# YaoTiancheng/DirectComputeRayTracing

Hardware: AMD Instinct MI355X
Metric: Mrays/s and ms/spp at 1920x1080, 8-bounce wavefront (higher is better)
Workload: dtype f32; 1 GPU; cornell_box_obj 1920x1080, 1733 spp (1 spp/step, film stripes across 1 GPU(s)), 8 bounces, wavefront, point light; spp=1733, max_bounce=8, streams_per_gpu=3, snapshot_spp=1733, parallelism=single GPU, 3 concurrent pipelines per GPU (cost-balanced bands), partition=balanced, interleave=False, bands_per_rank=3, rays=48252902736

## Files before the change

### directcomputeraytracing_amd/_abi.py

```python
from __future__ import annotations

import ctypes as C
import os
from pathlib import Path

PKG_DIR = Path(__file__).resolve().parent
LIB_PATH = PKG_DIR / "libdcrt.so"

DCRT_OK = 0
ABI_VERSION = 5
ERRORS = {-1: "DCRT_E_INVALID_ARG", -2: "DCRT_E_HIP", -3: "DCRT_E_NO_SCENE", -4: "DCRT_E_IO",
          -5: "DCRT_E_LIMIT", -6: "DCRT_E_NO_DEVICE"}
LIGHT_INDEX_INVALID = 0xFFFFFFFF
FEATURE_GGX_SAMPLE_VNDF = 0x01
FEATURE_NO_FRONT_TO_BACK = 0x02
FEATURE_LIGHT_VISIBLE = 0x04
FEATURE_WATERTIGHT = 0x08
FEATURE_ALLOW_ANYHIT = 0x10
FEATURE_DEFAULT = FEATURE_GGX_SAMPLE_VNDF | FEATURE_LIGHT_VISIBLE | FEATURE_WATERTIGHT
FILTER_BOX, FILTER_TRIANGLE, FILTER_GAUSSIAN, FILTER_MITCHELL, FILTER_LANCZOS = range(5)
MATERIAL_DIFFUSE, MATERIAL_PLASTIC, MATERIAL_CONDUCTOR, MATERIAL_DIELECTRIC, MATERIAL_THIN_DIELECTRIC = range(5)
MAX_LIGHT_COUNT = 5000
DIRTY_LIGHTS = 0x01
DIRTY_MATERIALS = 0x02
DIRTY_INSTANCE_FLAGS = 0x04
DIRTY_CAMERA = 0x08
DIRTY_SCENE = 0x10
(OUTPUT_PATH_TRACING, OUTPUT_SHADING_NORMAL, OUTPUT_SHADING_TANGENT, OUTPUT_ALBEDO, OUTPUT_NEGATIVE_NDOTV,
 OUTPUT_BACKFACE, OUTPUT_ITERATION_COUNT) = range(7)


class Vertex(C.Structure):
    _fields_ = [("position", C.c_float * 3), ("normal", C.c_float * 3), ("tangent", C.c_float * 3),
                ("texcoord", C.c_float * 2)]


class BVHNode(C.Structure):
    _fields_ = [("bbox_min", C.c_float * 3), ("bbox_max", C.c_float * 3), ("right_child_or_prim_index", C.c_uint32),
                ("misc", C.c_uint32)]


class Material(C.Structure):
    _fields_ = [("albedo", C.c_float * 3), ("albedo_texture_index", C.c_int32), ("ior", C.c_float * 3),
                ("roughness", C.c_float), ("tex_tiling", C.c_float * 2), ("opacity", C.c_float),
                ("flags", C.c_uint32), ("opacity_texture_index", C.c_int32)]


class Light(C.Structure):
    _fields_ = [("radiance", C.c_float * 3), ("position_or_triangle_range", C.c_float * 3), ("flags", C.c_uint32)]


class Float4x3(C.Structure):
    _fields_ = [("m", C.c_float * 12)]


class Texture(C.Structure):
    _fields_ = [("width", C.c_uint32), ("height", C.c_uint32), ("format", C.c_uint32),
                ("pixels", C.POINTER(C.c_uint8))]


class FlatScene(C.Structure):
    _fields_ = [
        ("vertices", C.POINTER(Vertex)), ("vertex_count", C.c_uint32),
        ("triangles", C.POINTER(C.c_uint32)), ("triangle_count", C.c_uint32),
        ("bvh_nodes", C.POINTER(BVHNode)), ("bvh_node_count", C.c_uint32),
        ("tlas_node_count", C.c_uint32),
        ("material_ids", C.POINTER(C.c_uint32)),
        ("instance_transforms", C.POINTER(Float4x3)), ("instance_count", C.c_uint32),
        ("instance_light_indices", C.POINTER(C.c_uint32)),
        ("instance_flags", C.POINTER(C.c_uint32)),
        ("instance_material_overrides", C.POINTER(C.c_uint32)),
        ("materials", C.POINTER(Material)), ("material_count", C.c_uint32),
        ("lights", C.POINTER(Light)), ("light_count", C.c_uint32),
        ("environment_light_index", C.c_uint32),
        ("textures", C.POINTER(Texture)), ("texture_count", C.c_uint32),
        ("env_cube_rgb", C.POINTER(C.c_float)), ("env_cube_size", C.c_uint32),
        ("bvh_traversal_stack_size", C.c_uint32),
    ]


class BxDFLuts(C.Structure):
    _fields_ = [("brdf", C.c_uint16 * (32 * 32)), ("brdf_avg", C.c_uint16 * 32),
                ("brdf_dielectric", C.c_uint16 * (32 * 16 * 32)), ("brdf_dielectric_avg", C.c_uint16 * (16 * 16 * 2)),
                ("bsdf", C.c_uint16 * (32 * 16 * 32)), ("bsdf_avg", C.c_uint16 * (16 * 16 * 2))]


class FrameParams(C.Structure):
    _fields_ = [("camera_transform", C.c_float * 16), ("resolution", C.c_uint32 * 2), ("film_size", C.c_float * 2),
                ("aperture_radius", C.c_float), ("focal_distance", C.c_float), ("film_distance", C.c_float),
                ("blade_count", C.c_uint32), ("blade_vertex_pos", C.c_float * 2), ("aperture_base_angle", C.c_float),
                ("frame_seed", C.c_uint32), ("max_bounce_count", C.c_uint32), ("light_count", C.c_uint32),
                ("environment_light_index", C.c_uint32), ("features", C.c_uint32)]


class FilterParams(C.Structure):
    _fields_ = [("filter", C.c_uint32), ("radius", C.c_float), ("gaussian_alpha", C.c_float),
                ("mitchell_b", C.c_float), ("mitchell_c", C.c_float), ("lanczos_tau", C.c_uint32)]


class Ray(C.Structure):
    _fields_ = [("origin", C.c_float * 3), ("t_max", C.c_float), ("direction", C.c_float * 3), ("t_min", C.c_float)]


class RayHit(C.Structure):
    _fields_ = [("t", C.c_float), ("u", C.c_float), ("v", C.c_float), ("triangle_id", C.c_uint32),
                ("instance_index", C.c_uint32)]


class PostFxParams(C.Structure):
    _fields_ = [("enabled", C.c_int32), ("auto_exposure", C.c_int32), ("ev100", C.c_float), ("luminance_white", C.c_float)]


class TracerConfig(C.Structure):
    _fields_ = [("path_pool_size", C.c_uint32), ("iterations_per_render", C.c_uint32), ("device", C.c_int32),
                ("stream", C.c_void_p), ("debug_rng", C.c_uint32)]


class OutputParams(C.Structure):
    _fields_ = [("output_type", C.c_uint32), ("iteration_threshold", C.c_uint32)]


class DenoiseParams(C.Structure):
    _fields_ = [("iterations", C.c_uint32), ("sigma_luminance", C.c_float), ("sigma_normal", C.c_float),
                ("sigma_albedo", C.c_float), ("demodulate", C.c_uint32)]


class NoiseStats(C.Structure):
    _fields_ = [("images", C.c_uint32), ("valid_pixels", C.c_uint32), ("converged_pixels", C.c_uint32),
                ("mean_error", C.c_float), ("max_error", C.c_float), ("max_tile_error", C.c_float)]


class ConvergeParams(C.Structure):
    _fields_ = [("threshold", C.c_float), ("target_fraction", C.c_float), ("min_images", C.c_uint32),
                ("max_images", C.c_uint32), ("check_interval", C.c_uint32)]


class AdaptiveReport(C.Structure):
    _fields_ = [("images", C.c_uint32), ("check_points", C.c_uint32), ("pixel_samples", C.c_uint64),
                ("active_blocks", C.c_uint32), ("total_blocks", C.c_uint32)]


class RayStats(C.Structure):
    _fields_ = [("extension_rays", C.c_uint64), ("shadow_rays", C.c_uint64), ("new_paths", C.c_uint64),
                ("iterations", C.c_uint64), ("images_completed", C.c_uint64)]


class FilmPartition(C.Structure):
    _fields_ = [("world_size", C.c_uint32), ("rank", C.c_uint32), ("stripe_height", C.c_uint32),
                ("halo_rows", C.c_uint32)]


class TraversalStats(C.Structure):
    _fields_ = [("ext_node_visits", C.c_uint64), ("ext_triangle_tests", C.c_uint64), ("ext_blas_entries", C.c_uint64),
                ("shadow_node_visits", C.c_uint64), ("shadow_triangle_tests", C.c_uint64),
                ("shadow_blas_entries", C.c_uint64), ("ext_launches", C.c_uint64), ("ext_kernel_ms", C.c_double),
                ("ext_max_node_visits", C.c_uint64), ("shadow_max_node_visits", C.c_uint64),
                ("material_launches", C.c_uint64), ("material_kernel_ms", C.c_double),
                ("control_launches", C.c_uint64), ("control_kernel_ms", C.c_double)]


class TracerInfo(C.Structure):
    _fields_ = [("path_pool_size", C.c_uint32), ("scene_in_lds", C.c_uint32), ("cached_nodes", C.c_uint32),
                ("cached_triangles", C.c_uint32), ("cast_block", C.c_uint32), ("traversal_stack", C.c_uint32),
                ("material_generic", C.c_uint32), ("pair_traversal", C.c_uint32), ("control_grid", C.c_uint32),
                ("material_grid", C.c_uint32), ("cast_grid", C.c_uint32), ("material_lds", C.c_uint32),
                ("cast_identity", C.c_uint32), ("stack_lds_rows", C.c_uint32), ("ring_rows", C.c_uint32),
                ("cast_waves_per_cu", C.c_uint32), ("shadow_cells", C.c_uint32), ("shadow_cell_max_leaves", C.c_uint32),
                ("shadow_cell_mean_leaves", C.c_float), ("shadow_inline", C.c_uint32), ("shading_tables", C.c_uint32),
                ("dielectric_row_bytes", C.c_uint32), ("dielectric_row_lds", C.c_uint32), ("frame_table_bytes", C.c_uint32)]


class ShadowCellsInfo(C.Structure):
    _fields_ = [("resolution", C.c_uint32), ("leaf_count", C.c_uint32), ("node_count", C.c_uint32),
                ("max_leaves", C.c_uint32), ("mean_leaves", C.c_float), ("r0", C.c_float)]


class UploadStats(C.Structure):
    _fields_ = [("scene_uploads", C.c_uint64), ("material_updates", C.c_uint64), ("light_updates", C.c_uint64),
                ("instance_flag_updates", C.c_uint64), ("geometry_bytes", C.c_uint64), ("shading_bytes", C.c_uint64),
                ("graph_invalidations", C.c_uint64)]


class MaterialSetting(C.Structure):
    _fields_ = [("albedo", C.c_float * 3), ("roughness", C.c_float), ("ior", C.c_float * 3), ("opacity", C.c_float),
                ("k", C.c_float * 3), ("tiling", C.c_float * 2), ("material_type", C.c_uint32),
                ("albedo_texture_index", C.c_int32), ("opacity_texture_index", C.c_int32),
                ("internal_scattering_mode", C.c_uint32), ("multiscattering", C.c_uint32),
                ("is_two_sided", C.c_uint32), ("has_roughness_texture", C.c_uint32)]


class SceneSettings(C.Structure):
    _fields_ = [("resolution", C.c_uint32 * 2), ("max_bounce_count", C.c_uint32), ("camera_type", C.c_uint32),
                ("fov_x", C.c_float), ("focal_length", C.c_float), ("focal_distance", C.c_float),
                ("relative_aperture", C.c_float), ("aperture_blade_count", C.c_uint32), ("aperture_rotation", C.c_float),
                ("film_size", C.c_float * 2), ("camera_position", C.c_float * 3), ("camera_euler_angles", C.c_float * 3),
                ("features", C.c_uint32), ("has_environment_light", C.c_uint32), ("environment_color", C.c_float * 3),
                ("env_cube_rgb", C.POINTER(C.c_float)), ("env_cube_size", C.c_uint32),
                ("mesh_light_count", C.c_uint32), ("punctual_light_count", C.c_uint32),
                ("material_count", C.c_uint32), ("texture_count", C.c_uint32)]


class ObjMesh(C.Structure):
    _fields_ = [("vertices", C.POINTER(Vertex)), ("vertex_count", C.c_uint32), ("indices", C.POINTER(C.c_uint32)),
                ("material_ids", C.POINTER(C.c_uint32)), ("triangle_count", C.c_uint32)]


class ObjMaterial(C.Structure):
    _fields_ = [("albedo", C.c_float * 3), ("ior", C.c_float), ("roughness", C.c_float), ("opacity", C.c_float),
                ("albedo_texture_index", C.c_int32), ("opacity_texture_index", C.c_int32)]


class BsdfProbeMaterial(C.Structure):
    _fields_ = [("type", C.c_uint32), ("albedo", C.c_float * 3), ("ior", C.c_float * 3), ("alpha", C.c_float),
                ("two_sided", C.c_uint32), ("multiscattering", C.c_uint32), ("internal_scattering_mode", C.c_uint32)]


OBJ_SCENE_LAYOUT = 1

_P = C.c_void_p
_I = C.c_int
_U = C.c_uint32
_FP = C.POINTER(C.c_float)
SIGNATURES = [
    ("dcrt_abi_version", _I, []),
    ("dcrt_version", C.c_char_p, []),
    ("dcrt_last_error", C.c_char_p, []),
    ("dcrt_device_count", _I, [C.POINTER(C.c_int)]),
    ("dcrt_scene_create", _I, [C.POINTER(_P)]),
    ("dcrt_scene_destroy", None, [_P]),
    ("dcrt_scene_reset", _I, [_P, _U, _U]),
    ("dcrt_scene_load_from_file", _I, [_P, C.c_char_p]),
    ("dcrt_scene_add_punctual_light", _I, [_P, _FP, _FP, _FP, _I]),
    ("dcrt_scene_set_punctual_light", _I, [_P, _U, _FP, _FP, _FP, _I]),
    ("dcrt_scene_remove_punctual_light", _I, [_P, _U]),
    ("dcrt_scene_remove_environment_light", _I, [_P]),
    ("dcrt_scene_acquire_dirty", _I, [_P, C.POINTER(C.c_uint32)]),
    ("dcrt_scene_flatten", _I, [_P]),
    ("dcrt_scene_set_environment_light", _I, [_P, _FP, _FP, _U]),
    ("dcrt_scene_set_camera", _I, [_P, _FP, _FP]),
    ("dcrt_scene_set_lens", _I, [_P, _I, C.c_float, C.c_float, C.c_float, C.c_float, _U, C.c_float, _FP]),
    ("dcrt_scene_set_max_bounce", _I, [_P, _U]),
    ("dcrt_scene_set_filter", _I, [_P, C.POINTER(FilterParams)]),
    ("dcrt_scene_get_filter", _I, [_P, C.POINTER(FilterParams)]),
    ("dcrt_scene_get_resolution", _I, [_P, C.POINTER(C.c_uint32), C.POINTER(C.c_uint32)]),
    ("dcrt_scene_get_material_count", _I, [_P, C.POINTER(C.c_uint32)]),
    ("dcrt_scene_set_material", _I, [_P, _U, _I, _FP, C.c_float, _FP, _FP, _I, _I]),
    ("dcrt_scene_set_material_opacity", _I, [_P, _U, C.c_float, C.c_int32]),
    ("dcrt_scene_get_material_setting", _I, [_P, _U, C.POINTER(MaterialSetting)]),
    ("dcrt_scene_set_material_multiscattering", _I, [_P, _U, _I]),
    ("dcrt_scene_get_settings", _I, [_P, C.POINTER(SceneSettings)]),
    ("dcrt_scene_get_mesh_light", _I, [_P, _U, C.POINTER(C.c_uint32), _FP]),
    ("dcrt_scene_get_punctual_light", _I, [_P, _U, _FP, _FP, _FP, C.POINTER(C.c_int)]),
# ... 155 lines not shown
```

### directcomputeraytracing_amd/csrc/device/dscene.h

```cpp
#pragma once

#include "../../../include/dcrt.h"
#include "dmath.h"
#include "../host/shadow_cells.h"

namespace dcrt {
namespace dev {

constexpr uint32_t kCapMatDiffuse = 1u << 0;
constexpr uint32_t kCapMatPlastic = 1u << 1;
constexpr uint32_t kCapMatConductor = 1u << 2;
constexpr uint32_t kCapMatDielectric = 1u << 3;
constexpr uint32_t kCapMatThin = 1u << 4;
constexpr uint32_t kCapMultiscatter = 1u << 5;
constexpr uint32_t kCapTextures = 1u << 6;
constexpr uint32_t kCapLightPoint = 1u << 7;
constexpr uint32_t kCapLightMesh = 1u << 8;
constexpr uint32_t kCapLightDirectional = 1u << 9;
constexpr uint32_t kCapLightEnv = 1u << 10;
constexpr uint32_t kCapEnvCube = 1u << 11;
constexpr uint32_t kCapAll = (1u << 12) - 1u;
constexpr uint32_t kCapEnvImportance = 1u << 12;
constexpr uint32_t kCapAllEnvImportance = kCapAll | kCapEnvImportance;
constexpr bool caps_any_scene(uint32_t caps) { return (caps & kCapAll) == kCapAll; }
constexpr uint32_t kCapMaterialsMask = 0x1Fu;
constexpr uint32_t kCapLightShift = 7;
constexpr uint32_t kCapOpaqueDelta = kCapMatDiffuse | kCapMatPlastic | kCapMatConductor | kCapLightPoint | kCapLightDirectional;

template <uint32_t CAPS>
DEV void assume_light_caps(uint32_t flags)
{
    if constexpr (!caps_any_scene(CAPS)) __builtin_assume((flags & ~((CAPS >> kCapLightShift) & 0xFu) & 0xFu) == 0u);
}

struct TextureDesc {
    uint32_t width, height, format, offset;
};

struct DeviceScene {
    const float4* nodes;
    const float4* triVerts;
    const float4* triShade;
    const dcrt_vertex* vertices;
    const uint32_t* triangles;
    const uint32_t* materialIds;
    const float4* transforms;
    const uint32_t* instanceLightIndices;
    const uint32_t* instanceFlags;
    const uint32_t* instanceIdentity;
    const uint32_t* overrides;
    const dcrt_material* materials;
    const dcrt_light* lights;
    const TextureDesc* textures;
    const uint8_t* texels;
    const float* srgbTable;
    const float* envCube;
    const uint16_t* lutBrdf;
    const uint16_t* lutBrdfAvg;
    const uint16_t* lutBrdfDielectric;
    const uint16_t* lutBrdfDielectricAvg;
    const uint16_t* lutBsdf;
    const uint16_t* lutBsdfAvg;
    uint32_t instanceCount;
    uint32_t nodeCount;
    uint32_t triangleCount;
    uint32_t envCubeSize;
    uint32_t stackSize;
    uint32_t stackRows;
    uint32_t ringRows;
    uint32_t* spill;
    uint32_t cachedNodes;
    uint32_t cachedTris;
    uint32_t cachedInstances;
    uint32_t singlePrimLeaves;
    uint32_t pairLayout;
    uint32_t skipRoot;
    uint32_t ldsMaterials, ldsLights;
    const uint64_t* shadowCells;
    const uint32_t* shadowLeaves;
    uint32_t shadowRes;
    const float* dielRows;
    uint32_t ldsRows;
    uint32_t shadingTables;
    const float4* triFrames;
    uint32_t ldsFrames;
    const float* envProb;
    const float* envRowCdf;
    const float* envMarginal;
};

constexpr uint32_t kTableDeltaPdf = 1u << 0;
constexpr uint32_t kTableDielRows = 1u << 1;
constexpr uint32_t kTableFrames = 1u << 2;
constexpr uint32_t kTableAll = kTableDeltaPdf | kTableDielRows | kTableFrames;
constexpr uint32_t kFrameFlatNormal = 1u, kFrameFlatTangent = 2u;
constexpr uint32_t kDielRowFloats = 132;
constexpr uint32_t kDielRowsMaxMaterials = 64;
constexpr __host__ __device__ uint32_t diel_rows_bytes(uint32_t materials) { return 4u * kDielRowFloats * materials; }

struct MaterialLds {
    uint32_t shading, rows, frames, cells;
    uint32_t framesAt, cellsAt;
    constexpr __host__ __device__ uint32_t Bytes(bool fused) const { return fused ? cellsAt + cells : frames ? framesAt + frames : shading + rows; }
};
constexpr __host__ __device__ MaterialLds material_lds_layout(uint32_t T, uint32_t I, uint32_t M, uint32_t L, uint32_t rowMaterials, bool frames,
                                                              uint32_t cellNodes, bool fused)
{
    MaterialLds l{};
    l.shading = 16u * (9u * T + 3u * I) + 4u * (2u * I + 13u * M + 7u * L);
    l.rows = diel_rows_bytes(rowMaterials);
    l.framesAt = (l.shading + l.rows + 15u) & ~15u;
    l.frames = frames ? 48u * T : 0u;
    l.cellsAt = (l.Bytes(false) + 15u) & ~15u;
    l.cells = fused ? 32u * cellNodes + 144u * T + 4u * kCellWords : 0u;
    return l;
}
static_assert(material_lds_layout(32, 8, 6, 1, 0, false, 0, false).shading == 5396u && material_lds_layout(32, 8, 6, 1, 0, false, 0, false).Bytes(false) == 5396u, "");
static_assert(material_lds_layout(32, 8, 6, 1, 6, false, 0, false).Bytes(false) == 8564u && material_lds_layout(32, 8, 6, 1, 6, true, 0, false).Bytes(false) == 8576u + 1536u, "");
static_assert(material_lds_layout(32, 8, 6, 1, 6, true, 40, true).cellsAt == 10112u && material_lds_layout(32, 8, 6, 1, 6, true, 40, true).Bytes(true) == 10112u + 5888u + 4u * kCellWords, "");
static_assert(material_lds_layout(32, 8, 6, 1, 0, false, 40, true).cellsAt == 5408u && material_lds_layout(32, 8, 6, 1, 6, false, 40, true).cellsAt == 8576u, "");
static_assert(material_lds_layout(0, 8, 6, 1, 0, false, 0, false).Bytes(false) == 788u && material_lds_layout(0, 8, 6, 1, 6, false, 0, false).Bytes(false) == 3956u, "");
static_assert(material_lds_layout(32, 8, 6, 3, 0, false, 0, false).shading == 5452u && material_lds_layout(32, 8, 6, 3, 0, true, 0, false).framesAt == 5456u, "");
static_assert(material_lds_layout(32, 8, 6, 3, 0, true, 40, true).cellsAt == 5456u + 1536u && material_lds_layout(32, 8, 6, 3, 0, false, 40, true).cellsAt == 5456u, "");

enum : int { kLayoutFlat = 0, kLayoutPairs = 1, kLayoutScene = 2 };
template <int LAYOUT>
DEV void node_children(const DeviceScene& sc, uint32_t node, uint32_t right, uint32_t* left, uint32_t* rightChild)
{
    const uint32_t r = right | (node & 0x80000000u);
    const bool pairs = LAYOUT == kLayoutPairs || (LAYOUT == kLayoutScene && sc.pairLayout != 0u);
    *left = pairs ? r : node + 1u;
    *rightChild = pairs ? r + 1u : r;
}


DEV float4* scene_cache(const DeviceScene& sc, uint32_t* stackMem, uint32_t shift)
{
    return (float4*)(stackMem + (sc.stackRows << shift));
}
typedef float LoadF4 __attribute__((ext_vector_type(4)));
DEV float4 lds_load4(const float4* genericLds, uint32_t i)
{
    const __attribute__((address_space(3))) LoadF4* p = (const __attribute__((address_space(3))) LoadF4*)(uint32_t)(uintptr_t)genericLds;
    const LoadF4 v = p[i];
    return make_float4(v.x, v.y, v.z, v.w);
}
DEV uint64_t global_load_u64(const uint64_t* g, size_t i)
{
    const __attribute__((address_space(1))) uint64_t* p = (const __attribute__((address_space(1))) uint64_t*)(uintptr_t)g;
    return p[i];
}
typedef float LoadF2 __attribute__((ext_vector_type(2)));
DEV float2 global_load2(const float2* g, size_t i)
{
    const __attribute__((address_space(1))) LoadF2* p = (const __attribute__((address_space(1))) LoadF2*)(uintptr_t)g;
    const LoadF2 v = p[i];
    return make_float2(v.x, v.y);
}
DEV float4 global_load4(const float4* g, size_t i)
{
    const __attribute__((address_space(1))) LoadF4* p = (const __attribute__((address_space(1))) LoadF4*)(uintptr_t)g;
    const LoadF4 v = p[i];
    return make_float4(v.x, v.y, v.z, v.w);
}
constexpr uint32_t kRotTriFloat4 = 9;
template <bool ROTATED>
DEV uint32_t cache_tri_float4() { return ROTATED ? kRotTriFloat4 : 3u; }
DEV float4 rot_tri_float4(const float4* triVerts, uint32_t i)
{
    const uint32_t tri = i / kRotTriFloat4, r = i - tri * kRotTriFloat4, z = r / 3u, k = r - z * 3u;
    const float4 q = triVerts[(size_t)tri * 3 + k];
// ... 1069 lines not shown
```

### directcomputeraytracing_amd/csrc/device/kernels.h

```cpp
#pragma once

#include "dbsdf.h"

namespace dcrt {
namespace dev {

constexpr uint32_t kFlagIdle = 0x80000000u;
constexpr uint32_t kFlagShadowRayHit = 0x40000000u;
constexpr uint32_t kFlagTerminate = 0x20000000u;
constexpr uint32_t kFlagDelta = 0x10000000u;
constexpr uint32_t kFlagFirst = 0x08000000u;
constexpr uint32_t kFlagShadowPending = 0x04000000u;
constexpr uint32_t kFlagShadowResolved = 0x02000000u;
constexpr uint32_t kBlockW = 8, kBlockH = 8;
#ifndef DCRT_CONTROL_BLOCK
#define DCRT_CONTROL_BLOCK 256
#endif
constexpr uint32_t kControlBlock = DCRT_CONTROL_BLOCK;
static_assert(kControlBlock % 64 == 0 && kControlBlock <= 960, "CONTROL workgroup: whole waves, at most 15");

constexpr uint32_t kShards = 8;
constexpr uint32_t kShardStride = 64;
constexpr uint32_t kQExt = 0, kQShadow = 1, kQFinish = 2, kQueues = 3;
#ifndef DCRT_FIN_SHARDS
#define DCRT_FIN_SHARDS 8
#endif
constexpr uint32_t kFinShards = DCRT_FIN_SHARDS;
constexpr uint32_t kCounterWords = 2 * kShards + kFinShards;
constexpr uint32_t kVirtualWord = kCounterWords;
constexpr uint32_t kNoPixel = 0xFFFFFFFFu;
constexpr uint32_t kDrainedWord = kCounterWords + 1;
constexpr uint32_t kInlineShadowWord = kCounterWords + 2;
constexpr uint32_t kCounterLines = kCounterWords + 2 + kShards;
constexpr uint32_t kEntryFirst = 0x80000000u;

struct Counters {
    uint32_t w[kCounterLines * kShardStride];
};
DEV uint32_t inline_shadow_rays(const Counters* c)
{
    uint32_t t = 0;
    for (uint32_t s = 0; s < kShards; ++s) t += c->w[(kInlineShadowWord + s) * kShardStride];
    return t;
}
DEV uint32_t virtual_items(const Counters* c) { return c->w[kVirtualWord * kShardStride]; }
DEV bool drained(const Counters* c) { return c->w[kDrainedWord * kShardStride] != 0u; }
struct Globals {
    uint32_t nextBlock[kShards * kShardStride];
    uint32_t totalBlocks;
    uint32_t stackOverflow;
    uint32_t imageComplete;
    uint32_t poolIdle;
    uint32_t prevLive;
    uint32_t stopped;
    uint32_t imagesDone, imageTarget, seedBase;
    uint32_t batchImages;
    uint32_t batchCap;
    uint32_t staticFill, staticGrid;
    uint32_t skipFilm;
    uint32_t filmImageBase;
    unsigned long long extRays, shadowRays, iterations;
};

DEV uint32_t* qctr(Counters* c, uint32_t q, uint32_t s) { return c->w + (q * kShards + s) * kShardStride; }
DEV uint32_t qctr_load(const Counters* c, uint32_t q, uint32_t s) { return c->w[(q * kShards + s) * kShardStride]; }
DEV uint32_t qtotal(const Counters* c, uint32_t q)
{
    uint32_t t = 0;
    for (uint32_t s = 0; s < kShards; ++s) t += qctr_load(c, q, s);
    return t;
}
template <uint32_t N = kShards>
struct QueueMapN {
    uint32_t prefix[N + 1];
};
using QueueMap = QueueMapN<kShards>;
template <uint32_t N>
DEV void qmap(const Counters* c, uint32_t q, QueueMapN<N>* m)
{
    m->prefix[0] = 0;
    for (uint32_t s = 0; s < N; ++s) m->prefix[s + 1] = m->prefix[s] + qctr_load(c, q, s);
}
template <uint32_t N>
DEV uint32_t qentry(const uint32_t* queue, uint32_t cap, const QueueMapN<N>& m, uint32_t i)
{
    uint32_t s = 0, base = 0;
#pragma unroll
    for (uint32_t k = 1; k < N; ++k) {
        const bool ge = i >= m.prefix[k];
        s += ge ? 1u : 0u;
        base = ge ? m.prefix[k] : base;
    }
    return queue[(size_t)s * cap + (i - base)];
}

template <uint32_t N>
DEV uint32_t qpos(uint32_t cap, const QueueMapN<N>& m, uint32_t i)
{
    uint32_t s = 0, base = 0;
#pragma unroll
    for (uint32_t k = 1; k < N; ++k) {
        const bool ge = i >= m.prefix[k];
        s += ge ? 1u : 0u;
        base = ge ? m.prefix[k] : base;
    }
    return s * cap + (i - base);
}
DEV float4* ext_rec(float4* recs, uint32_t q) { return (float4*)((char*)recs + (uint64_t)(q * 32u)); }
DEV const float4* ext_rec(const float4* recs, uint32_t q) { return (const float4*)((const char*)recs + (uint64_t)(q * 32u)); }

struct FrameConstants {
    float camera[16];
    uint32_t resolution[2];
    float filmSize[2];
    float apertureRadius, focalDistance, filmDistance;
    uint32_t bladeCount;
    float bladeVertexPos[2];
    float apertureBaseAngle;
    uint32_t frameSeed;
    uint32_t maxBounce, lightCount, envLightIndex, features;
    uint32_t blocksX, bandCount;
    uint32_t blocksPerImage;
    uint32_t refillLanes, parkLanes;
    uint32_t virtualStart;
    uint32_t drainPaths;
    uint32_t seedStride;
    uint32_t shadowInlineMask;
};

struct ShadowInline {
    const float4* nodes;
    const uint64_t* cells;
    const uint32_t* leaves;
    uint32_t nodeCount;
    uint32_t res;
};
DEV uint32_t image_seed(const FrameConstants& fc, uint32_t image) { return fc.frameSeed + __umul24(image, fc.seedStride); }

DEV void generate_ray(const FrameConstants& f, float fsx, float fsy, float a0, float a1, float a2, V3* origin, V3* direction)
{
    V3 filmPos = mk(-fsx + 0.5f, fsy - 0.5f, -f.filmDistance);
    filmPos.x = filmPos.x * f.filmSize[0];
    filmPos.y = filmPos.y * f.filmSize[1];
    V3 o = mk(0.0f, 0.0f, 0.0f);
    V3 d = normalize(-filmPos);
    if (f.apertureRadius > 0.0f) {
        float apx, apy;
        if (f.bladeCount <= 2) {
            concentric_disk(a0, a1, &apx, &apy);
            apx = apx * f.apertureRadius;
            apy = apy * f.apertureRadius;
        } else {
            const float s = sqrtf(a0);
            const float u = 1.0f - s, v = a1 * s;
            const float px = f.bladeVertexPos[0] * (u + v);
            const float py = f.bladeVertexPos[1] * u - f.bladeVertexPos[1] * v;
            const float n = floorf(a2 * (float)f.bladeCount);
            const float theta = n * (kPiMul2 / (float)f.bladeCount) + f.apertureBaseAngle;
            float st, ct;
            det_sincos(theta, &st, &ct);
            apx = px * ct - py * st;
            apy = py * ct + px * st;
        }
        const V3 focus = d * (f.focalDistance / d.z);
        o = mk(apx, apy, 0.0f);
        d = normalize(focus - o);
    }
    *origin = mul44(o, 1.0f, f.camera);
    *direction = mul44(d, 0.0f, f.camera);
}

struct F3 {
    float x, y, z;
};
struct alignas(4) F4u {
    float x, y, z, w;
};

template <typename T>
DEV T& slot(T* base, uint32_t i)
{
    return *(T*)((char*)base + (uint64_t)(i * (uint32_t)sizeof(T)));
}

template <typename T>
DEV T& sample_at(T* base, uint32_t i)
{
    return *(T*)((char*)base + (uint64_t)i * (uint64_t)sizeof(T));
}
typedef float GlobalF2 __attribute__((ext_vector_type(2)));
typedef float GlobalF4 __attribute__((ext_vector_type(4)));
DEV void store_global(float2* base, uint32_t i, float2 v)
{
    const GlobalF2 x = {v.x, v.y};
    *(__attribute__((address_space(1))) GlobalF2*)((uintptr_t)base + (uint64_t)i * 8u) = x;
}
DEV void store_global(float4* base, uint32_t i, float4 v)
{
    const GlobalF4 x = {v.x, v.y, v.z, v.w};
    *(__attribute__((address_space(1))) GlobalF4*)((uintptr_t)base + (uint64_t)i * 16u) = x;
}

struct PathStateA {
    uint4 rng;
    float4 lsrMisc;
};
struct PathStateB {
    float4 thr;
    float4 liLsr;
};
struct FinishRec {
    float4 liLsr;
    float4 lsrSlot;
};
constexpr uint32_t kDestFinish = 0x80000000u;

struct PathPool {
    float4* hit;
    float4* shRec;
    uint32_t* pixel;
    uint32_t* flags;
    float* extOpacity;
    float* shadowOpacity;
    float4* extRec;
    const float4* extPrevRec;
    PathStateA* stateA;
    PathStateB* stateB;
    const PathStateA* stateAPrev;
    const PathStateB* stateBPrev;
    uint32_t* shadowHit;
    const uint32_t* shadowHitPrev;
    uint32_t* shadowQueue;
    FinishRec* finRec;
    const FinishRec* finPrevRec;
    uint32_t* finHit;
    const uint32_t* finHitPrev;
    uint32_t size;
    uint32_t recCap;
    uint32_t finCap;
};
template <typename T>
DEV T& state_at(T* base, uint32_t q) { static_assert(sizeof(T) == 32, "state halves are 32 B"); return *(T*)((char*)base + (uint64_t)(q * 32u)); }

struct Film {
    float2* samplePosition;
    float4* sampleValue;
    uint4* debugRng;
    float4* accum;
    const uint32_t* rowY;
    const uint32_t* rowOwned;
    const uint32_t* blockList;
    uint32_t width, height, rowCount;
};

struct SampleOut {
    float2* samplePosition;
    float4* sampleValue;
    uint4* debugRng;
    uint32_t* rowRays;
};

DEV float2 pixel_sample(const FrameConstants& fc, uint32_t p)
{
    const uint32_t W = fc.resolution[0], wh = W * fc.resolution[1];
    const uint32_t image = p / wh, local = p - image * wh;
    const uint32_t py = local / W, px = local - py * W;
    Rng r = rng_init(px, py, image_seed(fc, image));
    const float psx = next1(r);
    const float psy = next1(r);
    return make_float2(psx, psy);
}

template <bool RAY>
DEV Rng new_path(const FrameConstants& fc, uint32_t p, V3* o, V3* d)
{
    const uint32_t W = fc.resolution[0], wh = W * fc.resolution[1];
    const uint32_t image = p / wh, local = p - image * wh;
    const uint32_t py = local / W, px = local - py * W;
    Rng rng = rng_init(px, py, image_seed(fc, image));
    const float psx = next1(rng), psy = next1(rng);
    const float a0 = next1(rng), a1 = next1(rng), a2 = next1(rng);
    if (RAY) {
        const float fsx = (psx + (float)px) / (float)fc.resolution[0];
        const float fsy = (psy + (float)py) / (float)fc.resolution[1];
        generate_ray(fc, fsx, fsy, a0, a1, a2, o, d);
    }
    return rng;
}

DEV bool block_pixel(const FrameConstants& fc, const Film& film, uint32_t block, uint32_t lane, uint32_t* px, uint32_t* py,
                     uint32_t* image)
{
    *image = block / fc.blocksPerImage;
    uint32_t local = block - *image * fc.blocksPerImage;
    if (film.blockList) local = film.blockList[local];
    const uint32_t band = local / fc.blocksX, bx = local - band * fc.blocksX;
    const uint32_t ri = band * kBlockH + lane / kBlockW;
// ... 9 lines not shown
```

### directcomputeraytracing_amd/csrc/device/kernels_impl.h

```cpp
#include "kernels.h"

namespace dcrt {
namespace dev {

#ifdef DCRT_PHASE_CLOCKS
__device__ unsigned long long g_phaseClk[24];
#define DCRT_PHASE_INIT unsigned long long clk_[6] = {0, 0, 0, 0, 0, 0}; unsigned long long tP_ = __builtin_amdgcn_s_memtime()
#define DCRT_PHASE(i) do { const unsigned long long t_ = __builtin_amdgcn_s_memtime(); clk_[i] += t_ - tP_; tP_ = t_; } while (0)
#define DCRT_PHASE_COUNT(i) (++clk_[i])
#define DCRT_PHASE_FLUSH() do { if ((threadIdx.x & 63u) == 0) for (int i_ = 0; i_ < 6; ++i_) atomicAdd(&g_phaseClk[i_], clk_[i_]); } while (0)
#define DCRT_MCLK_INIT unsigned long long mclk_[8] = {0, 0, 0, 0, 0, 0, 0, 0}; unsigned long long mT_ = __builtin_amdgcn_s_memtime()
#define DCRT_MCLK(i) do { const unsigned long long t_ = __builtin_amdgcn_s_memtime(); mclk_[i] += t_ - mT_; mT_ = t_; } while (0)
#define DCRT_MCLK_FLUSH(items) do { mclk_[7] += (items); if ((threadIdx.x & 63u) == 0) for (int i_ = 0; i_ < 8; ++i_) atomicAdd(&g_phaseClk[8 + i_], mclk_[i_]); } while (0)
#define DCRT_MCLK_PARAMS , unsigned long long (&mclk_)[8], unsigned long long& mT_
#define DCRT_MCLK_ARGS , mclk_, mT_
#else
#define DCRT_MCLK_PARAMS
#define DCRT_MCLK_ARGS
#define DCRT_MCLK_INIT do {} while (0)
#define DCRT_MCLK(i) do {} while (0)
#define DCRT_MCLK_FLUSH(items) do {} while (0)
#define DCRT_PHASE_INIT do {} while (0)
#define DCRT_PHASE(i) do {} while (0)
#define DCRT_PHASE_COUNT(i) do {} while (0)
// ... 154 lines not shown
    const size_t i = (size_t)blockIdx.x * blockDim.x + threadIdx.x;
    if (i >= (size_t)rows * n) return;
    const uint32_t r = (uint32_t)(i / n), x = (uint32_t)(i - (size_t)r * n);
    const uint32_t face = r / n, y = r - face * n;
    const double total = marginalSums[rows], rowTotal = rowTotals[r];
    prob[i] = (float)(env_texel_weight(cube, (int)n, (int)face, (int)y, (int)x) / total);
    rowCdf[i] = rowTotal > 0.0 ? (x == n - 1u ? 1.0f : (float)(rowSums[i] / rowTotal)) : 0.0f;
    if (x == 0u) marginal[r] = r == rows - 1u ? 1.0f : (float)(marginalSums[r] / total);
}

__global__ void build_diel_rows_kernel(const dcrt_material* materials, uint32_t count, const uint16_t* lut, const uint16_t* lutAvg,
                                       float* rows)
{
    const uint32_t i = blockIdx.x * blockDim.x + threadIdx.x;
    if (i >= count * kDielRowFloats) return;
    const uint32_t m = i / kDielRowFloats, k = i % kDielRowFloats;
    float roughness = materials[m].roughness;
    roughness = roughness * 1.0f;
    const float alpha = roughness * roughness;
    rows[i] = diel_row_value(lut, lutAvg, alpha, materials[m].ior[0], k);
}
__global__ void probe_diel_rows_kernel(const uint16_t* lut, const uint16_t* lutAvg, float* rows, float alpha, float ior)
{
    const uint32_t k = blockIdx.x * blockDim.x + threadIdx.x;
    if (k < kDielRowFloats) rows[k] = diel_row_value(lut, lutAvg, alpha, ior, k);
}

__global__ void build_tri_frames_kernel(const float4* triVerts, const float4* triShade, const float4* transforms, const uint32_t* triInstance,
                                        uint32_t count, float4* frames)
{
    const uint32_t t = blockIdx.x * blockDim.x + threadIdx.x;
    if (t >= count) return;
    const uint32_t inst = triInstance[t];
    float4 f0 = make_float4(0.0f, 0.0f, 0.0f, 0.0f), f1 = f0, f2 = f0;
    if (inst != 0xFFFFFFFFu) {
        const float4* P = triVerts + (size_t)t * 3;
        const float4* Q = triShade + (size_t)t * 6;
        const float4 q0 = P[0], q1 = P[1], q2 = P[2];
        const float4 a0 = Q[0], b0 = Q[1], a1 = Q[2], b1 = Q[3], a2 = Q[4], b2 = Q[5];
        const float4* M = transforms + (size_t)inst * 3;
        const V3 n = frame_normal(a0, a1, a2, 0.0f, 0.0f);
        const V3 nw = normalize(mul43(n, 0.0f, M));
        const V3 tw = normalize(mul43(frame_tangent(a0, b0, a1, b1, a2, b2, 0.0f, 0.0f, n), 0.0f, M));
        const V3 gw = normalize(mul43(frame_geometry_normal(mk(q0.x, q0.y, q0.z), mk(q1.x, q1.y, q1.z), mk(q2.x, q2.y, q2.z)), 0.0f, M));
        auto same3 = [](float x0, float y0, float z0, float x1, float y1, float z1) {
            return asu(x0) == asu(x1) && asu(y0) == asu(y1) && asu(z0) == asu(z1);
        };
        uint32_t flags = 0u;
        if (same3(a0.x, a0.y, a0.z, a1.x, a1.y, a1.z) && same3(a0.x, a0.y, a0.z, a2.x, a2.y, a2.z)) flags |= kFrameFlatNormal;
        if (same3(a0.w, b0.x, b0.y, a1.w, b1.x, b1.y) && same3(a0.w, b0.x, b0.y, a2.w, b2.x, b2.y)) flags |= kFrameFlatTangent;
        f0 = make_float4(nw.x, nw.y, nw.z, asf(flags));
        f1 = make_float4(tw.x, tw.y, tw.z, 0.0f);
        f2 = make_float4(gw.x, gw.y, gw.z, 0.0f);
    }
    frames[(size_t)t * 3] = f0;
    frames[(size_t)t * 3 + 1] = f1;
    frames[(size_t)t * 3 + 2] = f2;
}

__global__ void build_tri_verts_kernel(const dcrt_vertex* vertices, const uint32_t* triangles, const uint32_t* materialIds,
                                       uint32_t count, float4* out, float4* shade)
{
    const uint32_t t = blockIdx.x * blockDim.x + threadIdx.x;
    if (t >= count) return;
    V3 p[3];
    for (int k = 0; k < 3; ++k) {
        const dcrt_vertex& v = vertices[triangles[t * 3 + k]];
        p[k] = mk(v.position[0], v.position[1], v.position[2]);
        shade[(size_t)t * 6 + 2 * k] = make_float4(v.normal[0], v.normal[1], v.normal[2], v.tangent[0]);
        shade[(size_t)t * 6 + 2 * k + 1] = make_float4(v.tangent[1], v.tangent[2], v.texcoord[0], v.texcoord[1]);
    }
    const V3 cp = cross(p[1] - p[0], p[2] - p[0]);
    const float degenerate = dot(cp, cp) == 0.0f ? 1.0f : 0.0f;
    out[(size_t)t * 3] = make_float4(p[0].x, p[0].y, p[0].z, degenerate);
    out[(size_t)t * 3 + 1] = make_float4(p[1].x, p[1].y, p[1].z, __uint_as_float(materialIds[t]));
    out[(size_t)t * 3 + 2] = make_float4(p[2].x, p[2].y, p[2].z, 0.0f);
}

__global__ __launch_bounds__(kControlBlock) void control_kernel(PathPool pool, Film film, const FrameConstants* __restrict__ fc, Counters* cnt,
                                                       const Counters* prev, Globals* g, uint32_t debugRng)
{
    __shared__ uint32_t sm[64];
    if (g->stopped) return;
    {
        QueueMapN<kFinShards> fm;
        qmap(prev, kQFinish, &fm);
        const uint32_t nFin = drained(prev) ? 0u : fm.prefix[kFinShards];
        for (uint32_t i = blockIdx.x * blockDim.x + threadIdx.x; i < nFin; i += gridDim.x * blockDim.x) {
            const uint32_t f = qpos(pool.finCap, fm, i);
            const FinishRec fr = pool.finPrevRec[f];
            const bool shadowHit = pool.finHitPrev[f] != 0u;
            const uint32_t path = asu(fr.lsrSlot.z);
            F3 li{fr.liLsr.x, fr.liLsr.y, fr.liLsr.z};
            const F3 lsr{fr.liLsr.w, fr.lsrSlot.x, fr.lsrSlot.y};
            li.x = li.x + (!shadowHit ? lsr.x : 0.0f);
            li.y = li.y + (!shadowHit ? lsr.y : 0.0f);
            li.z = li.z + (!shadowHit ? lsr.z : 0.0f);
            const uint32_t p = slot(pool.pixel, path);
            sample_at(film.samplePosition, p) = pixel_sample(*fc, p);
            sample_at(film.sampleValue, p) = make_float4(li.x, li.y, li.z, 0.0f);
            slot(pool.flags, path) = kFlagIdle;
        }
    }
    const uint32_t lane = threadIdx.x & 63u;
    const uint32_t shard = blockIdx.x % kShards;
    uint32_t* cursor = &g->nextBlock[shard * kShardStride];
    const uint32_t shardBlocks = g->totalBlocks > shard ? (g->totalBlocks - shard + kShards - 1) / kShards : 0u;
    const bool staticFill = g->staticFill != 0u;
    if (staticFill && fc->virtualStart) {
        for (uint32_t base = blockIdx.x * blockDim.x; base < pool.size; base += gridDim.x * blockDim.x) {
            const uint32_t tid = base + threadIdx.x;
            const uint32_t vb = base / kControlBlock;
            const uint32_t claimed = (vb / kShards) * (kControlBlock >> 6) + (threadIdx.x >> 6);
            uint32_t pixel = kNoPixel, px = 0, py = 0, image = 0;
            if (claimed < shardBlocks && block_pixel(*fc, film, shard + claimed * kShards, lane, &px, &py, &image)) {
                pixel = image * (film.width * film.height) + py * film.width + px;
                pool.flags[tid] = 0u;
            }
            pool.pixel[tid] = pixel;
        }
        if (blockIdx.x == 0 && threadIdx.x == 0) cnt->w[kVirtualWord * kShardStride] = pool.size;
        return;
    }
    if (!staticFill) {
        __shared__ uint32_t exhausted;
        if (threadIdx.x == 0) exhausted = __hip_atomic_load(cursor, __ATOMIC_RELAXED, __HIP_MEMORY_SCOPE_AGENT) >= shardBlocks;
        __syncthreads();
        if (exhausted) return;
    }
    for (uint32_t base = blockIdx.x * blockDim.x; base < pool.size; base += gridDim.x * blockDim.x) {
    const uint32_t tid = base + threadIdx.x;
    const uint32_t vb = base / kControlBlock;
    const bool idle = (pool.flags[tid] & kFlagIdle) != 0;
    const bool waveIdle = __ballot(!idle) == 0ull;
    uint32_t claimed = 0;
    bool got = false;
    if (staticFill) {
        claimed = (vb / kShards) * (kControlBlock >> 6) + (threadIdx.x >> 6);
        got = waveIdle && claimed < shardBlocks;
    } else {
        bool want = false;
        if (waveIdle && lane == 0)
            want = __hip_atomic_load(cursor, __ATOMIC_RELAXED, __HIP_MEMORY_SCOPE_AGENT) < shardBlocks;
        uint32_t bslot, unused;
        block_append2(false, cursor, want, cursor, sm, &unused, &bslot);
        claimed = (uint32_t)__shfl((int)bslot, 0, 64);
        got = __shfl((int)want, 0, 64) != 0 && claimed < shardBlocks;
    }
    const uint32_t block = shard + claimed * kShards;
    bool newPath = false;
    V3 o = mk(0.0f, 0.0f, 0.0f), d = mk(0.0f, 0.0f, 0.0f);
    Rng rng;
    rng.s0 = rng.s1 = rng.s2 = rng.s3 = 0u;
    if (got) {
        uint32_t px = 0, py = 0, image = 0;
        if (block_pixel(*fc, film, block, lane, &px, &py, &image)) {
            rng = rng_init(px, py, image_seed(*fc, image));
            const float psx = next1(rng), psy = next1(rng);
            const float fsx = (psx + (float)px) / (float)fc->resolution[0];
            const float fsy = (psy + (float)py) / (float)fc->resolution[1];
            const float a0 = next1(rng), a1 = next1(rng), a2 = next1(rng);
            generate_ray(*fc, fsx, fsy, a0, a1, a2, &o, &d);
            if (fc->features & DCRT_FEATURE_ALLOW_ANYHIT) pool.extOpacity[tid] = next1(rng);
            pool.pixel[tid] = image * (film.width * film.height) + py * film.width + px;
            pool.flags[tid] = 0u;
            newPath = true;
        }
    }
    uint32_t eslot, unused;
    block_append2(newPath, qctr(cnt, kQExt, shard), false, qctr(cnt, kQExt, shard), sm + 32, &eslot, &unused);
    if (newPath) {
        const uint32_t q = shard * pool.recCap + eslot;
        float4* r = ext_rec(pool.extRec, q);
        r[0] = make_float4(o.x, o.y, o.z, 0.0f);
        r[1] = make_float4(d.x, d.y, d.z, asf(tid));
        PathStateA& st = state_at(pool.stateA, q);
        st.rng = make_uint4(rng.s0, rng.s1, rng.s2, rng.s3);
        st.lsrMisc = make_float4(0.0f, 0.0f, asf(kFlagDelta | kFlagFirst), asf(tid));
    }
    }
}

template <uint32_t CAPS, bool FRAMES = false>
__device__ __forceinline__ void shade_path(const DeviceScene& sc, const FrameConstants& fc, const HitRecord& hit, V3 dir, Rng& rng,
                                           uint32_t& flags, float4& thr, const F3& li, V3& T, V3& L, V3& lsr, bool& terminate,
                                           bool& hasShadow, V3& nO, V3& nD, float4& sO, V3& sD, float& extOpacity,
                                           float& shadowOpacity DCRT_MCLK_PARAMS)
{
    const uint32_t bounce = flags & 0xFFu;
    const uint32_t features = fc.features;
    const bool vndf = (features & DCRT_FEATURE_GGX_SAMPLE_VNDF) != 0;
    const bool hasHit = hit.t != inf();
    Intersection it;
    it.lightIndex = DCRT_LIGHT_INDEX_INVALID; it.triangleIndex = 0;
    it.geometryNormal = mk(0.0f, 0.0f, 0.0f);
    if (hasHit) hit_to_intersection<CAPS, FRAMES>(sc, hit, it);
    DCRT_MCLK(1);
    T = mk(thr.x, thr.y, thr.z);
    L = mk(li.x, li.y, li.z);
    {
        const uint32_t lightIndex = hasHit ? it.lightIndex : fc.envLightIndex;
        const bool visible = (features & DCRT_FEATURE_LIGHT_VISIBLE) != 0;
        if (visible ? lightIndex != DCRT_LIGHT_INDEX_INVALID : (bounce > 0 && lightIndex != DCRT_LIGHT_INDEX_INVALID)) {
            V3 radiance; float lightPdf;
            evaluate_light<CAPS>(sc, lightIndex, it.triangleIndex, it.geometryNormal, dir, hit.t, fc.lightCount, &radiance, &lightPdf);
            if (lightPdf > 0.0f) {
                const float weight = !(flags & kFlagDelta) ? power_heuristic(thr.w, lightPdf) : 1.0f;
                L = L + T * radiance * weight;
            }
        }
    }
    lsr = mk(0.0f, 0.0f, 0.0f);
    if (bounce > fc.maxBounce || !hasHit) {
        flags |= kFlagTerminate;
        terminate = true;
    } else {
        const V3 wo = -dir;
        const BsdfFrame bf = bsdf_frame(sc, wo, it);
        if (fc.lightCount != 0) {
            const LightSample ls = sample_light<CAPS>(sc, it.position, fc.lightCount, rng);
            if (any_pos(ls.radiance) && ls.pdf > 0.0f) {
                const V3 bsdf = evaluate_bsdf(sc, vndf, ls.wi, bf, it);
                const float NdotWI = fabsf(dot(it.normal, ls.wi));
                bool wantPdf = true;
                if constexpr ((CAPS & (kCapLightMesh | kCapLightEnv)) == 0u) wantPdf = (sc.shadingTables & kTableDeltaPdf) == 0u;
                float bsdfPdf = 0.0f;
                if (wantPdf) bsdfPdf = evaluate_bsdf_pdf(sc, vndf, ls.wi, bf, it);
                const float weight = ls.isDelta ? 1.0f : power_heuristic(ls.pdf, bsdfPdf);
                lsr = T * ls.radiance * bsdf * NdotWI * weight / ls.pdf;
                const V3 so = offset_ray_origin(it.position, it.geometryNormal, ls.wi);
                sO = make_float4(so.x, so.y, so.z, ls.distance);
                sD = ls.wi;
                hasShadow = true;
            }
        }
        DCRT_MCLK(3);
        float bsdfPdf = 0.0f;
        bool isDelta = false;
        {
            const float sel = next1(rng);
            const float sx = next1(rng), sy = next1(rng);
            V3 wi, bsdf;
            sample_bsdf(sc, vndf, bf, sx, sy, sel, it, &wi, &bsdf, &bsdfPdf, &isDelta);
            if ((bsdf.x != 0.0f || bsdf.y != 0.0f || bsdf.z != 0.0f) && bsdfPdf != 0.0f) {
                const float NdotWI = fabsf(dot(it.normal, wi));
                T = T * bsdf * NdotWI / bsdfPdf;
                nO = offset_ray_origin(it.position, it.geometryNormal, wi);
                nD = wi;
                flags = (flags & 0xFFFFFF00u) | ((bounce + 1) & 0xFFu);
            } else {
                flags |= kFlagTerminate;
                terminate = true;
            }
        }
        thr.w = bsdfPdf;
        flags = isDelta ? flags | kFlagDelta : flags & ~kFlagDelta;
        if (features & DCRT_FEATURE_ALLOW_ANYHIT) {
            if (!terminate) extOpacity = next1(rng);
            if (hasShadow) shadowOpacity = next1(rng);
        }
    }
}

#ifndef DCRT_MATERIAL_BLOCK
#define DCRT_MATERIAL_BLOCK 256
#endif
static_assert(DCRT_MATERIAL_BLOCK % 64 == 0 && DCRT_MATERIAL_BLOCK <= 960, "MATERIAL workgroup: whole waves, at most 15 (block_append3)");
#ifndef DCRT_MATERIAL_WAVES_PER_EU
#define DCRT_MATERIAL_WAVES_PER_EU 5
#endif
#ifndef DCRT_MATERIAL_OD_WAVES_PER_EU
#define DCRT_MATERIAL_OD_WAVES_PER_EU 1
#endif
#define DCRT_MATERIAL_OCCUPANCY __attribute__((amdgpu_waves_per_eu(caps_any_scene(CAPS) || FUSED ? DCRT_MATERIAL_WAVES_PER_EU : DCRT_MATERIAL_OD_WAVES_PER_EU, 8)))
template <uint32_t CAPS, int SCENE_LDS, bool PROBE = false, bool FUSED = false>
__global__ __launch_bounds__(DCRT_MATERIAL_BLOCK) DCRT_MATERIAL_OCCUPANCY void material_kernel(PathPool pool, DeviceScene sc, const FrameConstants* __restrict__ fcr, Counters* cnt,
                                                                             const Counters* prev, const SampleOut* __restrict__ sampleOut, ShadowInline si)
{
    static_assert(!FUSED || (SCENE_LDS == 1 && !PROBE), "FUSED: beside the whole LDS shading copy");
#if defined(DCRT_MATERIAL_PRIO) && DCRT_MATERIAL_PRIO > 0
    __builtin_amdgcn_s_setprio(DCRT_MATERIAL_PRIO);
#endif
    __shared__ uint32_t sm[96 + (FUSED ? 1 : 0)];
    QueueMap qm;
    qmap(prev, kQExt, &qm);
    const uint32_t virt = virtual_items(prev);
    const uint32_t count = drained(prev) ? 0u : (virt ? virt : qm.prefix[kShards]);
    const uint32_t shard = blockIdx.x % kShards;
    const uint32_t fshard = blockIdx.x % kFinShards;
    const FrameConstants& fcv = *fcr;
    const float4* cellNodes = nullptr;
    const float4* cellTris = nullptr;
    const uint32_t* cellLeaves = nullptr;
    uint32_t& inlineTotal = sm[FUSED ? 96 : 0];
    uint32_t inlineRays = 0;
    if constexpr (SCENE_LDS != 0) {
        extern __shared__ float4 sceneLds[];
        if (blockIdx.x * blockDim.x >= count) return;
        const uint32_t T = SCENE_LDS == 1 ? sc.triangleCount : 0u, I = sc.instanceCount;
        float4* tv = sceneLds;
        float4* ts = tv + 3u * T;
        float4* tf = ts + 6u * T;
        uint32_t* w = (uint32_t*)(tf + 3u * I);
        uint32_t* li = w;
        uint32_t* ov = li + I;
        uint32_t* mt = ov + I;
        uint32_t* lt = mt + 13u * sc.ldsMaterials;
        float* rw = (float*)(lt + 7u * sc.ldsLights);
        for (uint32_t i = threadIdx.x; i < kDielRowFloats * sc.ldsRows; i += blockDim.x) rw[i] = sc.dielRows[i];
        const uint32_t frameOff = material_lds_layout(T, I, sc.ldsMaterials, sc.ldsLights, sc.ldsRows, false, 0u, false).framesAt;
        const uint32_t FT = sc.ldsFrames ? T : 0u;
        float4* fr = sceneLds + (frameOff >> 4);
        for (uint32_t i = threadIdx.x; i < 3u * FT; i += blockDim.x) fr[i] = sc.triFrames[i];
        for (uint32_t i = threadIdx.x; i < 3u * T; i += blockDim.x) tv[i] = sc.triVerts[i];
        for (uint32_t i = threadIdx.x; i < 6u * T; i += blockDim.x) ts[i] = sc.triShade[i];
        for (uint32_t i = threadIdx.x; i < 3u * I; i += blockDim.x) tf[i] = sc.transforms[i];
        for (uint32_t i = threadIdx.x; i < I; i += blockDim.x) { li[i] = sc.instanceLightIndices[i]; ov[i] = sc.overrides[i]; }
        for (uint32_t i = threadIdx.x; i < 13u * sc.ldsMaterials; i += blockDim.x) mt[i] = ((const uint32_t*)sc.materials)[i];
        for (uint32_t i = threadIdx.x; i < 7u * sc.ldsLights; i += blockDim.x) lt[i] = ((const uint32_t*)sc.lights)[i];
        if constexpr (FUSED) {
            float4* cn = fr + 3u * FT;
            float4* ct = cn + 2u * si.nodeCount;
            uint32_t* cl = (uint32_t*)(ct + kRotTriFloat4 * T);
            for (uint32_t i = threadIdx.x; i < 2u * si.nodeCount; i += blockDim.x) cn[i] = si.nodes[i];
            for (uint32_t i = threadIdx.x; i < kRotTriFloat4 * T; i += blockDim.x) ct[i] = rot_tri_float4(sc.triVerts, i);
            for (uint32_t i = threadIdx.x; i < kCellWords; i += blockDim.x) cl[i] = si.leaves[i];
            if (threadIdx.x == 0) inlineTotal = 0u;
            cellNodes = cn;
            cellTris = ct;
            cellLeaves = cl;
        }
        __syncthreads();
        if constexpr (SCENE_LDS == 1) {
            sc.triVerts = tv;
            sc.triShade = ts;
        }
        sc.transforms = tf;
        sc.instanceLightIndices = li;
        sc.overrides = ov;
        sc.materials = (const dcrt_material*)mt;
        sc.lights = (const dcrt_light*)lt;
        if (sc.ldsRows != 0u) sc.dielRows = rw;
        if (FT != 0u) sc.triFrames = fr;
    }
    DCRT_MCLK_INIT;
    uint32_t itemsDone = 0;
    uint32_t round = 0;
    for (uint32_t base = blockIdx.x * blockDim.x; base < count; base += gridDim.x * blockDim.x) {
    const uint32_t i = base + threadIdx.x;
    bool active = i < count;
    uint32_t newPixel = kNoPixel;
    if (virt && active) {
        newPixel = slot(pool.pixel, i);
        active = newPixel != kNoPixel;
    }
    bool terminate = false, hasShadow = false, ends = false;
    uint32_t path = 0, pix = 0;
    float4 sample = make_float4(0.0f, 0.0f, 0.0f, 0.0f);
    float2* outPos = nullptr;
    float4* outVal = nullptr;
    V3 nO = mk(0.0f, 0.0f, 0.0f), nD = mk(0.0f, 0.0f, 0.0f);
    float4 sO = make_float4(0.0f, 0.0f, 0.0f, 0.0f);
    V3 sD = mk(0.0f, 0.0f, 0.0f);
    uint32_t pathFlags = 0;
    float4 sThr = make_float4(0.0f, 0.0f, 0.0f, 0.0f);
    V3 sT = mk(0.0f, 0.0f, 0.0f), sL = mk(0.0f, 0.0f, 0.0f), sLsr = mk(0.0f, 0.0f, 0.0f);
    uint4 sRng = make_uint4(0u, 0u, 0u, 0u);
    if (active) {
        ++itemsDone;
        const float4 h4 = pool.hit[2 * i], hd = pool.hit[2 * i + 1];
        HitRecord hit;
        hit.t = h4.x; hit.u = h4.y; hit.v = h4.z; hit.tri = asu(h4.w); hit.inst = asu(hd.w);
        const V3 dir = mk(hd.x, hd.y, hd.z);
        Rng rng;
        uint32_t flags;
        float4 thr, l4, l2;
        bool shadowHit = false;
        if (virt) {
            V3 unusedO, unusedD;
            rng = new_path<false>(fcv, newPixel, &unusedO, &unusedD);
            path = i;
            flags = kFlagDelta;
            thr = make_float4(1.0f, 1.0f, 1.0f, 0.0f);
            l4 = make_float4(0.0f, 0.0f, 0.0f, 0.0f);
            l2 = make_float4(0.0f, 0.0f, 0.0f, 0.0f);
        } else {
            const uint32_t q = qpos(pool.recCap, qm, i);
            const PathStateA& ps = state_at(pool.stateAPrev, q);
            const PathStateB& psB = state_at(pool.stateBPrev, q);
            const uint4 r4 = ps.rng;
            l2 = ps.lsrMisc;
            const float4 bThr = psB.thr, bLi = psB.liLsr;
            uint32_t shRaw = 0u;
            if constexpr (FUSED) {
                if (__ballot((asu(l2.z) & kFlagShadowPending) != 0u) != 0ull) shRaw = pool.shadowHitPrev[q];
            } else {
                shRaw = pool.shadowHitPrev[q];
            }
            rng.s0 = r4.x; rng.s1 = r4.y; rng.s2 = r4.z; rng.s3 = r4.w;
            path = asu(l2.w);
            flags = asu(l2.z);
            const bool first = (flags & kFlagFirst) != 0u;
            thr = first ? make_float4(1.0f, 1.0f, 1.0f, 0.0f) : bThr;
            l4 = first ? make_float4(0.0f, 0.0f, 0.0f, 0.0f) : bLi;
            shadowHit = (flags & kFlagShadowResolved) != 0u || ((flags & kFlagShadowPending) != 0u && shRaw != 0u);
            flags &= ~(kFlagFirst | kFlagShadowPending | kFlagShadowResolved);
        }
        F3 li{l4.x, l4.y, l4.z};
        {
            const F3 lsr0{l4.w, l2.x, l2.y};
            li.x = li.x + (!shadowHit ? lsr0.x : 0.0f);
            li.y = li.y + (!shadowHit ? lsr0.y : 0.0f);
            li.z = li.z + (!shadowHit ? lsr0.z : 0.0f);
        }
        uint32_t out = path;
        asm volatile("" : "+v"(out));
        float extOpacity = 0.0f, shadowOpacity = 0.0f;
        V3 T, L, lsr;
        DCRT_MCLK(0);
        shade_path<CAPS, SCENE_LDS == 1 && !caps_any_scene(CAPS)>(sc, fcv, hit, dir, rng, flags, thr, li, T, L, lsr, terminate, hasShadow, nO, nD, sO, sD,
                         extOpacity, shadowOpacity DCRT_MCLK_ARGS);
        DCRT_MCLK(4);
        if (fcv.features & DCRT_FEATURE_ALLOW_ANYHIT) {
            if (!terminate) slot(pool.extOpacity, out) = extOpacity;
            if (hasShadow) slot(pool.shadowOpacity, out) = shadowOpacity;
        }
        ends = terminate && !hasShadow;
        if constexpr (PROBE) {
            uint32_t* rowRays = sampleOut->rowRays;
            const uint32_t p = virt ? newPixel : slot(pool.pixel, out);
            const uint32_t W = fcv.resolution[0], wh = W * fcv.resolution[1];
            atomicAdd(&rowRays[(p % wh) / W], hasShadow ? 2u : 1u);
        }
        pathFlags = flags;
        sThr = thr;
        sT = T;
        sL = L;
        sLsr = lsr;
        sRng = make_uint4(rng.s0, rng.s1, rng.s2, rng.s3);
        if (ends || terminate) {
            const SampleOut so = *sampleOut;
            if (ends || so.debugRng) pix = slot(pool.pixel, out);
            if (ends) {
                sample = make_float4(L.x + 0.0f, L.y + 0.0f, L.z + 0.0f, 0.0f);
                outPos = so.samplePosition;
                outVal = so.sampleValue;
            }
            if (so.debugRng) sample_at(so.debugRng, pix) = make_uint4(rng.s0, rng.s1, rng.s2, rng.s3);
        }
    }
    bool inlined = false, occluded = false;
    if constexpr (FUSED) {
        const V3 sInv = inv_dir(sD);
        inlined = active && hasShadow && cells_finite(sInv) && (path & fcv.shadowInlineMask) == 0u;
        if (inlined)
            occluded = cells_occluded_cached(si.cells, si.res, mk(sO.x, sO.y, sO.z), sD, sO.w, sInv,
                                             (fcv.features & DCRT_FEATURE_WATERTIGHT) != 0, cellNodes, cellTris, cellLeaves);
        inlineRays += (uint32_t)__popcll(__ballot(inlined));
    }
    const bool queued = active && hasShadow && !inlined;
    DCRT_MCLK(5);
    uint32_t es, ss;
    const bool fin = active && terminate && hasShadow;
    uint32_t fb;
    block_append3(active && !terminate, qctr(cnt, kQExt, shard), queued, qctr(cnt, kQShadow, shard),
                  fin, qctr(cnt, kQFinish, fshard), sm + (round & 1u) * 48u, &es, &ss, &fb);
    DCRT_MCLK(6);
    const uint32_t qNext = shard * pool.recCap + es;
    const uint32_t fPos = fshard * pool.finCap + fb;
    asm volatile("" ::"v"(pix));
    if (ends) {
        store_global(outPos, pix, pixel_sample(fcv, pix));
        store_global(outVal, pix, sample);
        slot(pool.flags, path) = kFlagIdle;
    }
    if (active && !terminate) {
        float4* r = ext_rec(pool.extRec, qNext);
        r[0] = make_float4(nO.x, nO.y, nO.z, 0.0f);
        r[1] = make_float4(nD.x, nD.y, nD.z, asf(path));
        PathStateA& st = state_at(pool.stateA, qNext);
        PathStateB& stB = state_at(pool.stateB, qNext);
        st.rng = sRng;
        stB.thr = make_float4(sT.x, sT.y, sT.z, sThr.w);
        stB.liLsr = make_float4(sL.x, sL.y, sL.z, sLsr.x);
        st.lsrMisc = make_float4(sLsr.y, sLsr.z, asf(pathFlags | (queued ? kFlagShadowPending : 0u) | (occluded ? kFlagShadowResolved : 0u)), asf(path));
    }
    if (fin) {
        FinishRec& fr = pool.finRec[fPos];
        fr.liLsr = make_float4(sL.x, sL.y, sL.z, sLsr.x);
        fr.lsrSlot = make_float4(sLsr.y, sLsr.z, asf(path), 0.0f);
        if (inlined) pool.finHit[fPos] = occluded ? 1u : 0u;
    }
    if (queued) {
        const uint32_t sq = shard * pool.recCap + ss;
        float4* r = ext_rec(pool.shRec, sq);
        r[0] = sO;
        r[1] = make_float4(sD.x, sD.y, sD.z, asf(terminate ? (fPos | kDestFinish) : qNext));
        if (fcv.features & DCRT_FEATURE_ALLOW_ANYHIT) slot(pool.shadowQueue, sq) = path;
    }
    DCRT_MCLK(2);
    ++round;
    }
    if constexpr (FUSED) {
        if ((threadIdx.x & 63u) == 0u && inlineRays) atomicAdd(&inlineTotal, inlineRays);
        __syncthreads();
        if (threadIdx.x == 0 && inlineTotal) atomicAdd(&cnt->w[(kInlineShadowWord + shard) * kShardStride], inlineTotal);
    }
    DCRT_MCLK_FLUSH(itemsDone);
    (void)itemsDone;
}

#ifndef DCRT_CAST_WAVES_PER_EU
#define DCRT_CAST_WAVES_PER_EU 5
#endif
#if DCRT_CAST_WAVES_PER_EU > 0
#define DCRT_CAST_OCCUPANCY __attribute__((amdgpu_waves_per_eu(DCRT_CAST_WAVES_PER_EU, 8)))
#else
#define DCRT_CAST_OCCUPANCY
#endif
#ifndef DCRT_CACHED_CAST_WAVES_PER_EU
#define DCRT_CACHED_CAST_WAVES_PER_EU 7
#endif


__device__ __forceinline__ uint32_t block_shift() { return 31u - (uint32_t)__clz((int)blockDim.x); }

#ifndef DCRT_VISITS_PER_CHECK
#define DCRT_VISITS_PER_CHECK 3
#endif
constexpr int kVisitsPerCheck = DCRT_VISITS_PER_CHECK;
#ifndef DCRT_INTERLEAVE
#define DCRT_INTERLEAVE 64
#endif
constexpr uint32_t kInterleave = DCRT_INTERLEAVE;

#ifdef DCRT_WAVE_TIMELINE
__device__ unsigned long long g_waveLog[2][16][8192][2];
__device__ uint32_t g_waveItems[2][16][8192];
#define DCRT_WAVE_TAG(g) ((int)((g)->iterations & 15ull))
#else
#define DCRT_WAVE_TAG(g) (-1)
#endif


constexpr uint32_t kNoItem = 0xFFFFFFFFu;
#ifndef DCRT_INLINE_ENTRY
#define DCRT_INLINE_ENTRY 1
#endif

constexpr uint32_t kMinRingRows = 2u * ((uint32_t)kVisitsPerCheck + 1u);
template <bool RING>
__device__ __forceinline__ void ring_maintain(const DeviceScene& sc, TravState& s, bool active, uint32_t* lds, uint32_t shift)
{
    if constexpr (RING) {
        const uint32_t stride = 4u << shift;
        const uint32_t live = s.sp - s.base;
        const bool spill = active && live > (sc.ringRows - (uint32_t)kVisitsPerCheck) * stride;
        const bool fill = active && s.base != 0u && live <= (uint32_t)kVisitsPerCheck * stride;
        if (__builtin_expect(__ballot(spill | fill) != 0ull, 0)) {
            const uint32_t lanes = gridDim.x * blockDim.x;
            uint32_t* col = sc.spill + (size_t)blockIdx.x * blockDim.x + threadIdx.x;
            const uint32_t half = (sc.ringRows >> 1) * stride;
            const uint32_t target = s.sp > half ? s.sp - half : 0u;
            if (spill) {
                for (uint32_t p = s.base + stride; p <= target; p += stride)
                    col[(size_t)((p >> (shift + 2u)) - 1u) * lanes] = stack_at(lds, stack_row<true>(sc, p, shift));
                s.base = target;
            } else if (fill) {
                for (uint32_t p = target + stride; p <= s.base; p += stride)
                    stack_at(lds, stack_row<true>(sc, p, shift)) = col[(size_t)((p >> (shift + 2u)) - 1u) * lanes];
                s.base = target;
            }
        }
    }
}

template <bool ANY_HIT, bool INSTR, bool OPACITY, bool LANE_ANY = false, bool ALL_CACHED = false, bool PAIR = false,
          int LAYOUT = kLayoutScene, bool IDENT = false, bool RING = false, bool FLAT = false, typename Lookup, typename Fetch,
          typename Emit>
__device__ __forceinline__ void persistent_trace(const DeviceScene& sc, uint32_t n, uint32_t features, uint32_t kRefillLanes,
                                                 uint32_t kParkLanes, uint32_t* lds, uint32_t shift, Lookup lookup, Fetch fetch,
                                                 Emit emit, TraversalStats& st, int waveTag = -1)
{
    const bool watertight = (features & DCRT_FEATURE_WATERTIGHT) != 0;
    const bool f2b = (features & DCRT_FEATURE_NO_FRONT_TO_BACK) == 0;
    const uint32_t wavesPerBlock = blockDim.x >> 6;
    const uint32_t lane = threadIdx.x & 63u;
    const uint32_t waves = gridDim.x * wavesPerBlock;
    const uint32_t waveId = blockIdx.x * wavesPerBlock + (threadIdx.x >> 6);
#ifndef DCRT_ADAPTIVE_GROUPS
#define DCRT_ADAPTIVE_GROUPS 1
#endif
    constexpr uint32_t kLgInterleave = 31u - __builtin_clz(kInterleave);
    const uint32_t perWave4 = n / (4u * waves);
    const uint32_t lg = !DCRT_ADAPTIVE_GROUPS || perWave4 >= kInterleave ? kLgInterleave : (perWave4 ? 31u - (uint32_t)__clz((int)perWave4) : 0u);
    const uint32_t gmask = (1u << lg) - 1u;
    const uint32_t groups = (n + gmask) >> lg;
    const uint32_t myGroups = groups > waveId ? (groups - waveId + waves - 1) / waves : 0u;
    uint32_t cursor = 0;
    const uint32_t end = myGroups << lg;
    const uint32_t chunk = end;
    auto itemIndex = [&](uint32_t k) { return ((waveId + __umul24(k >> lg, waves)) << lg) + (k & gmask); };
    TravState s;
    constexpr uint32_t kIdle = 0, kRun = 1, kPark = 2, kFin = 3;
    uint32_t ls = kIdle;
    uint32_t item = 0;
#ifdef DCRT_WAVE_TIMELINE
    const unsigned long long tStart = wall_clock64();
#endif
    DCRT_PHASE_INIT;
    for (;;) {
        DCRT_PHASE_COUNT(3);
        const bool free = ls == kIdle || ls == kFin;
        const unsigned long long need = __ballot(free);
        const uint32_t nNeed = (uint32_t)__popcll(need);
        const bool refill = nNeed >= kRefillLanes && cursor < end;
        const uint32_t k = cursor + __builtin_amdgcn_mbcnt_hi((uint32_t)(need >> 32), __builtin_amdgcn_mbcnt_lo((uint32_t)need, 0u));
        if (ls == kFin) {
            emit(item, s);
            ls = kIdle;
        }
        if (refill) {
            const uint32_t idx = itemIndex(k);
            if (free && k < end && idx < n) {
                item = fetch(idx, lookup(idx), s);
                if (!f2b) s.negMask = 0u;
                if constexpr (!INSTR && !PAIR && !RING && !OPACITY) {
                    if (sc.skipRoot && item != kNoItem) trav_skip_root<ALL_CACHED, LAYOUT, IDENT>(sc, s, lds, shift);
// ... 11 lines not shown
#pragma unroll
            for (int k = 0; k < kVisitsPerCheck; ++k) {
                if (ls == kRun) {
                    const bool fin = PAIR && !INSTR && !ALL_CACHED ? trav_visit_pair<false, LAYOUT, RING>(sc, s, lds, shift)
                                                                   : trav_visit<INSTR, ALL_CACHED, LAYOUT, !FLAT && (ALL_CACHED || IDENT) && !OPACITY && DCRT_INLINE_ENTRY, IDENT, RING>(sc, s, lds, shift, st);
                    if (fin) ls = kFin;
                    else if (s.parked) ls = kPark;
                }
            }
            const unsigned long long runnable = __ballot(ls == kRun);
            const uint32_t parked = (uint32_t)__popcll(__ballot(ls == kPark));
            const uint32_t idle = 64u - (uint32_t)__popcll(runnable) - parked;
            DCRT_PHASE_COUNT(4);
#ifndef DCRT_ADAPTIVE_PARK
#define DCRT_ADAPTIVE_PARK 1
#endif
#ifndef DCRT_PARK_EIGHTHS
#define DCRT_PARK_EIGHTHS 4
#endif
            const uint32_t parkAt = DCRT_ADAPTIVE_PARK ? min(kParkLanes, max(1u, ((64u - idle) * DCRT_PARK_EIGHTHS) >> 3)) : kParkLanes;
            if (runnable == 0ull || parked >= parkAt || (idle >= kRefillLanes && cursor < end)) break;
        }
        DCRT_PHASE(1);
        if (__ballot(ls == kPark) != 0ull) DCRT_PHASE_COUNT(5);
        if (ls == kPark)
            ls = trav_leaf<ANY_HIT, INSTR, OPACITY, LANE_ANY, ALL_CACHED, IDENT, RING, FLAT>(sc, s, watertight, lds, shift, st) ? kFin : kRun;
        DCRT_PHASE(2);
    }
    DCRT_PHASE_FLUSH();
#ifdef DCRT_WAVE_TIMELINE
    if (waveTag >= 0 && n > 0 && (threadIdx.x & 63u) == 0 && waveId < 8192) {
        g_waveLog[ANY_HIT ? 1 : 0][waveTag & 15][waveId][0] = tStart;
        g_waveLog[ANY_HIT ? 1 : 0][waveTag & 15][waveId][1] = wall_clock64();
        g_waveItems[ANY_HIT ? 1 : 0][waveTag & 15][waveId] = chunk;
    }
#endif
}

template <typename T>
__device__ __forceinline__ T* sgpr_ptr(T* p)
{
#if defined(__HIP_DEVICE_COMPILE__)
    __attribute__((address_space(1))) T* g = (__attribute__((address_space(1))) T*)p;
    asm volatile("" : "+s"(g));
    return (T*)g;
#else
    return p;
#endif
}

__device__ __forceinline__ void flush_stats(const TraversalStats& st, unsigned long long* dst)
{
    const unsigned long long a = wave_sum(st.nodes), b = wave_sum(st.tris), c = wave_sum(st.blas);
    if ((threadIdx.x & 63u) == 0 && (a | b | c)) { atomicAdd(&dst[0], a); atomicAdd(&dst[1], b); atomicAdd(&dst[2], c); }
}

__device__ __forceinline__ void flush_max(uint32_t v, unsigned long long* dst)
{
    for (int o = 32; o > 0; o >>= 1) v = max(v, (uint32_t)__shfl_xor((int)v, o, 64));
    if ((threadIdx.x & 63u) == 0 && v) atomicMax(dst, (unsigned long long)v);
}

__device__ __forceinline__ void emit_hit(const PathPool& pool, uint32_t item, const TravState& s)
{
    float4* h = pool.hit + 2 * (size_t)item;
    h[0] = s.found ? make_float4(s.hit.t, s.hit.u, s.hit.v, asf(s.hit.tri)) : make_float4(inf(), 0.0f, 0.0f, 0.0f);
    h[1] = make_float4(s.d.x, s.d.y, s.d.z, asf(s.found ? s.hit.inst : 0u));
}
__device__ __forceinline__ void emit_occlusion(const PathPool& pool, uint32_t dest, bool found)
{
    uint32_t* dst = (dest & kDestFinish) ? pool.finHit : pool.shadowHit;
    dst[dest & ~kDestFinish] = found ? 1u : 0u;
}
__device__ __forceinline__ void emit_occlusion(const PathPool& pool, uint32_t dest, const TravState& s) { emit_occlusion(pool, dest, s.found); }

template <bool INSTR, bool OPACITY>
__global__ __launch_bounds__(256) DCRT_CAST_OCCUPANCY void extension_kernel(PathPool pool, DeviceScene sc, const FrameConstants* __restrict__ fc, const Counters* cnt,
                                                         Globals* g, unsigned long long* instr)
{
    extern __shared__ uint32_t stackMem[];
    scene_cache_load(sc, stackMem, block_shift());
    QueueMap qm;
    qmap(cnt, kQExt, &qm);
    TraversalStats st = {};
    persistent_trace<false, INSTR, OPACITY>(
        sc, qm.prefix[kShards], fc->features, fc->refillLanes, fc->parkLanes, stackMem + threadIdx.x, block_shift(),
        [&](uint32_t i) __attribute__((always_inline)) { return qpos(pool.recCap, qm, i); },
        [&](uint32_t i, uint32_t q, TravState& s) __attribute__((always_inline)) {
            const float4* r = ext_rec((const float4*)pool.extRec, q);
            const float4 o = r[0], d = r[1];
            trav_init(s, mk(o.x, o.y, o.z), mk(d.x, d.y, d.z), 0.0f, inf());
            if (OPACITY) s.opacitySample = pool.extOpacity[asu(d.w) & ~kEntryFirst];
            return i;
        },
        [&](uint32_t item, const TravState& s) __attribute__((always_inline)) { emit_hit(pool, item, s); },
        st, DCRT_WAVE_TAG(g));
    if (INSTR) flush_stats(st, instr);
    (void)g;
}

__device__ __forceinline__ void end_iteration(const Counters* cnt, Counters* nextCnt, Globals* g, uint32_t shadowRays)
{
    if (blockIdx.x == 0) {
        if (threadIdx.x == 0) {
            uint32_t fin = 0;
            for (uint32_t sh = 0; sh < kFinShards; ++sh) fin += qctr_load(cnt, kQFinish, sh);
            const uint32_t virt = virtual_items(cnt);
            const uint32_t ext = virt ? virt : qtotal(cnt, kQExt);
            if (!virt) g->extRays += ext;
            g->shadowRays += shadowRays + inline_shadow_rays(cnt);
            g->iterations += 1ull;
            g->staticFill = 0u;
            const bool idle = g->prevLive == 0u && ext == 0u;
            g->poolIdle = idle ? 1u : 0u;
            g->imageComplete = (idle && !g->stopped) ? 1u : 0u;
            g->prevLive = ext + fin;
        }
        if (threadIdx.x < kCounterLines) nextCnt->w[threadIdx.x * kShardStride] = 0u;
    }
}

template <bool INSTR, bool OPACITY>
__global__ __launch_bounds__(256) DCRT_CAST_OCCUPANCY void shadow_kernel(PathPool pool, DeviceScene sc, const FrameConstants* __restrict__ fc, Counters* cnt,
                                                      Counters* nextCnt, Globals* g, unsigned long long* instr)
{
    extern __shared__ uint32_t stackMem[];
    scene_cache_load(sc, stackMem, block_shift());
    QueueMap qm;
    qmap(cnt, kQShadow, &qm);
    const uint32_t n = qm.prefix[kShards];
    TraversalStats st = {};
    persistent_trace<true, INSTR, OPACITY>(
        sc, n, fc->features, fc->refillLanes, fc->parkLanes, stackMem + threadIdx.x, block_shift(),
        [&](uint32_t i) __attribute__((always_inline)) { return qpos(pool.recCap, qm, i); },
        [&](uint32_t i, uint32_t q, TravState& s) __attribute__((always_inline)) {
            const float4* r = ext_rec((const float4*)pool.shRec, q);
            const float4 o = r[0], d = r[1];
            trav_init(s, mk(o.x, o.y, o.z), mk(d.x, d.y, d.z), 0.0f, o.w);
            if (OPACITY) s.opacitySample = pool.shadowOpacity[slot(pool.shadowQueue, q)];
            return asu(d.w);
        },
        [&](uint32_t dest, const TravState& s) __attribute__((always_inline)) { emit_occlusion(pool, dest, s); },
        st, DCRT_WAVE_TAG(g));
    if (INSTR) flush_stats(st, instr + 3);
    end_iteration(cnt, nextCnt, g, n);
}

#ifndef DCRT_IDENT_CAST_WAVES_PER_EU
#define DCRT_IDENT_CAST_WAVES_PER_EU 8
#endif
template <bool INSTR, bool OPACITY, bool ALL_CACHED, bool PAIR, bool IDENT = false, bool RING = false, bool FLAT = false,
          bool CELLS = false>
__global__ __launch_bounds__(256)
#ifndef DCRT_GLOBAL_CAST_WAVES_PER_EU
#define DCRT_GLOBAL_CAST_WAVES_PER_EU DCRT_CAST_WAVES_PER_EU
#endif
__attribute__((amdgpu_waves_per_eu(ALL_CACHED && !OPACITY && !INSTR ? (IDENT ? DCRT_IDENT_CAST_WAVES_PER_EU : DCRT_CACHED_CAST_WAVES_PER_EU)
                                   : (!ALL_CACHED && !PAIR && !OPACITY && !INSTR ? DCRT_GLOBAL_CAST_WAVES_PER_EU : DCRT_CAST_WAVES_PER_EU), 8))) void cast_kernel(PathPool pool, DeviceScene sc, const FrameConstants* __restrict__ fc, Counters* cnt,
                                                                     Counters* nextCnt, Globals* g, unsigned long long* instr)
{
    extern __shared__ uint32_t stackMem[];
    static_assert(!CELLS || (FLAT && ALL_CACHED && IDENT && !INSTR && !OPACITY && !PAIR && !RING), "CELLS: the entry-free cache-only kernel");
    uint32_t* leafWords = (uint32_t*)(scene_cache(sc, stackMem, block_shift()) + sc.cachedNodes * 2u + sc.cachedTris * kRotTriFloat4);
    if (CELLS && threadIdx.x < kCellWords) leafWords[threadIdx.x] = sc.shadowLeaves[threadIdx.x];
    scene_cache_load<ALL_CACHED>(sc, stackMem, block_shift());
    QueueMap qe, qs;
    qmap(cnt, kQExt, &qe);
    qmap(cnt, kQShadow, &qs);
    const uint32_t nExt = qe.prefix[kShards], nShadow = qs.prefix[kShards];
    const uint32_t* shQueue = sgpr_ptr(pool.shadowQueue);
    const float4* extRec = sgpr_ptr((const float4*)pool.extRec);
    const float4* shRec = sgpr_ptr((const float4*)pool.shRec);
    TraversalStats st = {};
    TraversalStats stExt = {}, stShadow = {};
    constexpr int kLayout = PAIR ? kLayoutPairs : (!INSTR || ALL_CACHED ? kLayoutFlat : kLayoutScene);
    const uint32_t virt = !OPACITY ? virtual_items(cnt) : 0u;
    if (!OPACITY && virt) {
        const FrameConstants& f = *fc;
        const uint32_t* pixels = sgpr_ptr((const uint32_t*)pool.pixel);
        uint32_t rays = 0;
        persistent_trace<false, INSTR, OPACITY, true, ALL_CACHED, PAIR, kLayout, IDENT, RING, FLAT>(
            sc, virt, f.features, f.refillLanes, f.parkLanes, stackMem + threadIdx.x, block_shift(),
            [&](uint32_t i) __attribute__((always_inline)) { return i; },
            [&](uint32_t i, uint32_t v, TravState& s) __attribute__((always_inline)) {
                const uint32_t p = slot(pixels, v);
                if (p == kNoPixel) return kNoItem;
                V3 o, d;
                (void)new_path<true>(f, p, &o, &d);
                trav_init(s, o, d, 0.0f, inf());
                s.anyHit = false;
                if (INSTR) st = TraversalStats{};
                ++rays;
                return i;
            },
            [&](uint32_t item, const TravState& s) __attribute__((always_inline)) {
                emit_hit(pool, item, s);
                if (INSTR) {
                    stExt.nodes += st.nodes; stExt.tris += st.tris; stExt.blas += st.blas;
                    stExt.maxNodes = max(stExt.maxNodes, st.nodes);
                }
            },
            st, DCRT_WAVE_TAG(g));
        const unsigned long long r = wave_sum(rays);
        if ((threadIdx.x & 63u) == 0 && r) atomicAdd(&g->extRays, r);
    } else if constexpr (CELLS) {
        const uint32_t wavesPerBlock = blockDim.x >> 6, waves = gridDim.x * wavesPerBlock;
        const uint32_t waveId = blockIdx.x * wavesPerBlock + (threadIdx.x >> 6);
        const bool watertight = (fc->features & DCRT_FEATURE_WATERTIGHT) != 0;
        auto shadowSection = [&]() __attribute__((always_inline)) {
            for (uint32_t i = (waveId << 6) + (threadIdx.x & 63u); i < nShadow; i += waves << 6) {
                const float4* r = ext_rec(shRec, qpos(pool.recCap, qs, i));
                const float4 o = r[0], d = r[1];
                emit_occlusion(pool, asu(d.w), cells_occluded(sc, o, d, watertight, stackMem + threadIdx.x, block_shift(), leafWords));
            }
        };
#ifndef DCRT_CELLS_LAST
#define DCRT_CELLS_LAST 0
#endif
        if (!DCRT_CELLS_LAST) shadowSection();
        persistent_trace<false, INSTR, OPACITY, false, ALL_CACHED, PAIR, kLayout, IDENT, RING, FLAT>(
            sc, nExt, fc->features, fc->refillLanes, fc->parkLanes, stackMem + threadIdx.x, block_shift(),
            [&](uint32_t i) __attribute__((always_inline)) { return qpos(pool.recCap, qe, i); },
            [&](uint32_t i, uint32_t v, TravState& s) __attribute__((always_inline)) {
                const float4* r = ext_rec(extRec, v);
                const float4 o = r[0], d = r[1];
                trav_init(s, mk(o.x, o.y, o.z), mk(d.x, d.y, d.z), 0.0f, inf());
                return i;
            },
            [&](uint32_t item, const TravState& s) __attribute__((always_inline)) { emit_hit(pool, item, s); },
            st, DCRT_WAVE_TAG(g));
        if (DCRT_CELLS_LAST) shadowSection();
    } else {
    persistent_trace<false, INSTR, OPACITY, true, ALL_CACHED, PAIR, kLayout, IDENT, RING, FLAT>(
        sc, nExt + nShadow, fc->features, fc->refillLanes, fc->parkLanes, stackMem + threadIdx.x, block_shift(),
        [&](uint32_t i) __attribute__((always_inline)) {
            return i >= nExt ? qpos(pool.recCap, qs, i - nExt) : qpos(pool.recCap, qe, i);
        },
        [&](uint32_t i, uint32_t v, TravState& s) __attribute__((always_inline)) {
            const bool shadow = i >= nExt;
            const float4* r = ext_rec(shadow ? shRec : extRec, v);
            const float4 o = r[0], d = r[1];
            trav_init(s, mk(o.x, o.y, o.z), mk(d.x, d.y, d.z), 0.0f, shadow ? o.w : inf());
            s.anyHit = shadow;
            if (OPACITY) {
                const uint32_t path = shadow ? slot(shQueue, v) : asu(d.w);
                s.opacitySample = shadow ? pool.shadowOpacity[path] : pool.extOpacity[path];
            }
            if (INSTR) st = TraversalStats{};
            return shadow ? asu(d.w) : i;
        },
        [&](uint32_t item, const TravState& s) __attribute__((always_inline)) {
            if (s.anyHit) emit_occlusion(pool, item, s);
            else emit_hit(pool, item, s);
            if (INSTR) {
                TraversalStats& dst = s.anyHit ? stShadow : stExt;
                dst.nodes += st.nodes; dst.tris += st.tris; dst.blas += st.blas;
                dst.maxNodes = max(dst.maxNodes, st.nodes);
#ifdef DCRT_PHASE_CLOCKS
                dst.cached += st.cached; dst.deep4 += st.deep4; dst.deep8 += st.deep8; dst.deep12 += st.deep12;
#endif
            }
        },
        st, DCRT_WAVE_TAG(g));
    }
    if (INSTR) {
        flush_stats(stExt, instr);
        flush_stats(stShadow, instr + 3);
        flush_max(stExt.maxNodes, instr + 6);
        flush_max(stShadow.maxNodes, instr + 7);
    }
#ifdef DCRT_PHASE_CLOCKS
    if (INSTR) {
        const unsigned long long c = wave_sum(stExt.cached + stShadow.cached), d4 = wave_sum(stExt.deep4 + stShadow.deep4),
                                 d8 = wave_sum(stExt.deep8 + stShadow.deep8), d12 = wave_sum(stExt.deep12 + stShadow.deep12);
        if ((threadIdx.x & 63u) == 0) {
            atomicAdd(&g_phaseClk[16], c); atomicAdd(&g_phaseClk[17], d4); atomicAdd(&g_phaseClk[18], d8); atomicAdd(&g_phaseClk[19], d12);
        }
    }
#endif
    end_iteration(cnt, nextCnt, g, nShadow);
}

template <bool ANY_HIT, bool OPACITY>
__device__ __forceinline__ bool trace_full(const DeviceScene& sc, V3 o, V3 d, float tMax, bool watertight, bool f2b,
                                           float opacitySample, uint32_t* lds, uint32_t shift, HitRecord* hit)
{
    TravState s;
    trav_init(s, o, d, 0.0f, tMax, f2b);
    s.opacitySample = opacitySample;
    TraversalStats st = {};
    for (;;) {
        if (trav_visit_pair(sc, s, lds, shift)) break;
        if (s.parked && trav_leaf<ANY_HIT, false, OPACITY>(sc, s, watertight, lds, shift, st)) break;
    }
    *hit = s.hit;
    return s.found;
}

template <bool OPACITY, uint32_t CAPS = kCapAll>
__global__ __launch_bounds__(256) void megakernel(DeviceScene sc, const FrameConstants* __restrict__ fcp, Film film, Globals* g, uint32_t debugRng)
{
    extern __shared__ uint32_t stackMem[];
    scene_cache_load(sc, stackMem, block_shift());
    __shared__ uint32_t sm[64];
    const FrameConstants& fc = *fcp;
    const uint32_t lane = threadIdx.x & 63u;
    const uint32_t shard = blockIdx.x % kShards;
    uint32_t* cursor = &g->nextBlock[shard * kShardStride];
    const uint32_t shardBlocks = g->totalBlocks > shard ? (g->totalBlocks - shard + kShards - 1) / kShards : 0u;
    const bool watertight = (fc.features & DCRT_FEATURE_WATERTIGHT) != 0;
    const bool f2b = (fc.features & DCRT_FEATURE_NO_FRONT_TO_BACK) == 0;
    const bool vndf = (fc.features & DCRT_FEATURE_GGX_SAMPLE_VNDF) != 0;
    const bool lightVisible = (fc.features & DCRT_FEATURE_LIGHT_VISIBLE) != 0;
    uint32_t* lds = stackMem + threadIdx.x;
    const uint32_t shift = block_shift();
    unsigned long long extRays = 0, shadowRays = 0;
    for (;;) {
        bool want = false;
        if (lane == 0) want = __hip_atomic_load(cursor, __ATOMIC_RELAXED, __HIP_MEMORY_SCOPE_AGENT) < shardBlocks;
        const uint32_t bslot = block_append(want, cursor, sm);
        const uint32_t claimed = (uint32_t)__shfl((int)bslot, 0, 64);
        const bool got = __shfl((int)want, 0, 64) != 0 && claimed < shardBlocks;
        if (__syncthreads_or(got ? 1 : 0) == 0) break;
        if (!got) continue;
        const uint32_t block = shard + claimed * kShards;
        uint32_t px = 0, py = 0, image = 0;
        if (!block_pixel(fc, film, block, lane, &px, &py, &image)) continue;
        Rng rng = rng_init(px, py, image_seed(fc, image));
        const float psx = next1(rng), psy = next1(rng);
        const float fsx = (psx + (float)px) / (float)fc.resolution[0];
        const float fsy = (psy + (float)py) / (float)fc.resolution[1];
        const float a0 = next1(rng), a1 = next1(rng), a2 = next1(rng);
        V3 ro, rd;
        generate_ray(fc, fsx, fsy, a0, a1, a2, &ro, &rd);
        V3 T = mk(1.0f, 1.0f, 1.0f), L = mk(0.0f, 0.0f, 0.0f);
        float bsdfPdfPrev = 0.0f;
// ... 88 lines not shown
}

template <bool OPACITY>
__global__ __launch_bounds__(256) void view_kernel(DeviceScene sc, const FrameConstants* __restrict__ fcp, Film film, Globals* g, uint32_t debugRng,
                                                   uint32_t outputType, uint32_t iterationThreshold)
{
    extern __shared__ uint32_t stackMem[];
    scene_cache_load(sc, stackMem, block_shift());
    __shared__ uint32_t sm[64];
    const FrameConstants& fc = *fcp;
    const uint32_t lane = threadIdx.x & 63u;
    const uint32_t shard = blockIdx.x % kShards;
    uint32_t* cursor = &g->nextBlock[shard * kShardStride];
    const uint32_t shardBlocks = g->totalBlocks > shard ? (g->totalBlocks - shard + kShards - 1) / kShards : 0u;
    const bool watertight = (fc.features & DCRT_FEATURE_WATERTIGHT) != 0;
    const bool f2b = (fc.features & DCRT_FEATURE_NO_FRONT_TO_BACK) == 0;
    uint32_t* lds = stackMem + threadIdx.x;
    const uint32_t shift = block_shift();
    uint32_t extRays = 0;
    for (;;) {
        bool want = false;
        if (lane == 0) want = __hip_atomic_load(cursor, __ATOMIC_RELAXED, __HIP_MEMORY_SCOPE_AGENT) < shardBlocks;
        const uint32_t bslot = block_append(want, cursor, sm);
        const uint32_t claimed = (uint32_t)__shfl((int)bslot, 0, 64);
        const bool got = __shfl((int)want, 0, 64) != 0 && claimed < shardBlocks;
        if (__syncthreads_or(got ? 1 : 0) == 0) break;
        if (!got) continue;
        const uint32_t block = shard + claimed * kShards;
        uint32_t px = 0, py = 0, image = 0;
        if (!block_pixel(fc, film, block, lane, &px, &py, &image)) continue;
        Rng rng = rng_init(px, py, image_seed(fc, image));
        const float psx = next1(rng), psy = next1(rng);
        const float fsx = (psx + (float)px) / (float)fc.resolution[0];
        const float fsy = (psy + (float)py) / (float)fc.resolution[1];
        const float a0 = next1(rng), a1 = next1(rng), a2 = next1(rng);
        V3 ro, rd;
        generate_ray(fc, fsx, fsy, a0, a1, a2, &ro, &rd);
        ++extRays;
        TravState s;
        trav_init(s, ro, rd, 0.0f, inf(), f2b);
        s.opacitySample = OPACITY ? next1(rng) : 0.0f;
        TraversalStats st = {};
        for (;;) {
            if (trav_visit<true>(sc, s, lds, shift, st)) break;
            if (s.parked && trav_leaf<false, true, OPACITY>(sc, s, watertight, lds, shift, st)) break;
        }
        V3 l = mk(0.0f, 0.0f, 0.0f);
        if (outputType == DCRT_OUTPUT_ITERATION_COUNT) {
            const float f = (float)st.nodes / (float)iterationThreshold;
            l = st.nodes <= iterationThreshold ? mk(f, f, f) : mk(1.0f, 0.0f, 0.0f);
        } else if (s.found) {
            Intersection it;
            hit_to_intersection(sc, s.hit, it);
            const V3 green = mk(0.0f, 1.0f, 0.0f), red = mk(1.0f, 0.0f, 0.0f);
            switch (outputType) {
            case DCRT_OUTPUT_SHADING_NORMAL: l = it.normal * 0.5f + mk(0.5f, 0.5f, 0.5f); break;
            case DCRT_OUTPUT_SHADING_TANGENT: l = it.tangent * 0.5f + mk(0.5f, 0.5f, 0.5f); break;
            case DCRT_OUTPUT_ALBEDO: l = it.albedo; break;
            case DCRT_OUTPUT_NEGATIVE_NDOTV: l = dot(-rd, it.normal) < 0.0f ? green : red; break;
            case DCRT_OUTPUT_BACKFACE: l = it.backface ? green : red; break;
            default: break;
            }
        }
        const size_t p = (size_t)image * film.width * film.height + (size_t)py * film.width + px;
        film.samplePosition[p] = make_float2(psx, psy);
        film.sampleValue[p] = make_float4(l.x, l.y, l.z, 0.0f);
        if (debugRng) film.debugRng[p] = make_uint4(rng.s0, rng.s1, rng.s2, rng.s3);
    }
    const unsigned long long e = wave_sum(extRays);
    if (lane == 0) atomicAdd(&g->extRays, e);
}

template <uint32_t CAPS>
__global__ __launch_bounds__(256) void drain_kernel(PathPool pool, DeviceScene sc, const FrameConstants* __restrict__ fcp, Counters* cnt,
                                                    Globals* g, const SampleOut* __restrict__ sampleOut)
{
    const FrameConstants& fc = *fcp;
    if (!fc.drainPaths || g->stopped || virtual_items(cnt)) return;
    QueueMap qe;
    qmap(cnt, kQExt, &qe);
    QueueMapN<kFinShards> fm;
    qmap(cnt, kQFinish, &fm);
    const uint32_t nExt = qe.prefix[kShards], nFin = fm.prefix[kFinShards];
    if (nExt + nFin == 0u || nExt + nFin > fc.drainPaths) return;
    for (uint32_t sh = 0; sh < kShards; ++sh) {
        const uint32_t blocks = g->totalBlocks > sh ? (g->totalBlocks - sh + kShards - 1) / kShards : 0u;
        if (__hip_atomic_load(&g->nextBlock[sh * kShardStride], __ATOMIC_RELAXED, __HIP_MEMORY_SCOPE_AGENT) < blocks) return;
    }
    extern __shared__ uint32_t stackMem[];
    scene_cache_load(sc, stackMem, block_shift());
    if (blockIdx.x == 0 && threadIdx.x == 0) {
        cnt->w[kDrainedWord * kShardStride] = 1u;
        g->prevLive = 0u;
    }
    const bool watertight = (fc.features & DCRT_FEATURE_WATERTIGHT) != 0;
    const bool f2b = (fc.features & DCRT_FEATURE_NO_FRONT_TO_BACK) == 0;
    uint32_t* lds = stackMem + threadIdx.x;
    const uint32_t shift = block_shift();
    const SampleOut so = *sampleOut;
    uint32_t extRays = 0, shadowRays = 0;
    const uint32_t waves = gridDim.x * (blockDim.x >> 6);
    const uint32_t wave = blockIdx.x * (blockDim.x >> 6) + (threadIdx.x >> 6);
    for (uint32_t w = (threadIdx.x & 63u) * waves + wave; w < nExt + nFin; w += 64u * waves) {
        if (w >= nExt) {
            const uint32_t f = qpos(pool.finCap, fm, w - nExt);
            const FinishRec fr = pool.finRec[f];
            const bool shadowHit = pool.finHit[f] != 0u;
            const uint32_t path = asu(fr.lsrSlot.z);
            F3 li{fr.liLsr.x, fr.liLsr.y, fr.liLsr.z};
            const F3 lsr{fr.liLsr.w, fr.lsrSlot.x, fr.lsrSlot.y};
            li.x = li.x + (!shadowHit ? lsr.x : 0.0f);
            li.y = li.y + (!shadowHit ? lsr.y : 0.0f);
            li.z = li.z + (!shadowHit ? lsr.z : 0.0f);
            const uint32_t p = slot(pool.pixel, path);
            sample_at(so.samplePosition, p) = pixel_sample(fc, p);
            sample_at(so.sampleValue, p) = make_float4(li.x, li.y, li.z, 0.0f);
            slot(pool.flags, path) = kFlagIdle;
            continue;
        }
        const uint32_t q = qpos(pool.recCap, qe, w);
        const PathStateA ps = state_at(pool.stateA, q);
        const float4 h4 = pool.hit[2 * w], hd = pool.hit[2 * w + 1];
        HitRecord hit;
        hit.t = h4.x; hit.u = h4.y; hit.v = h4.z; hit.tri = asu(h4.w); hit.inst = asu(hd.w);
        V3 dir = mk(hd.x, hd.y, hd.z);
        Rng rng;
        rng.s0 = ps.rng.x; rng.s1 = ps.rng.y; rng.s2 = ps.rng.z; rng.s3 = ps.rng.w;
        const uint32_t path = asu(ps.lsrMisc.w);
        uint32_t flags = asu(ps.lsrMisc.z);
        const bool first = (flags & kFlagFirst) != 0u;
        float4 thr = make_float4(1.0f, 1.0f, 1.0f, 0.0f), l4 = make_float4(0.0f, 0.0f, 0.0f, 0.0f);
        if (!first) {
            const PathStateB psB = state_at(pool.stateB, q);
            thr = psB.thr;
            l4 = psB.liLsr;
        }
        bool shadowHit = (flags & kFlagShadowResolved) != 0u || ((flags & kFlagShadowPending) ? pool.shadowHit[q] != 0u : false);
        flags &= ~(kFlagFirst | kFlagShadowPending | kFlagShadowResolved);
        F3 li{l4.x, l4.y, l4.z};
        V3 lsr0 = mk(l4.w, ps.lsrMisc.x, ps.lsrMisc.y);
        for (;;) {
            li.x = li.x + (!shadowHit ? lsr0.x : 0.0f);
            li.y = li.y + (!shadowHit ? lsr0.y : 0.0f);
            li.z = li.z + (!shadowHit ? lsr0.z : 0.0f);
            bool terminate = false, hasShadow = false;
            V3 T, L, lsr, nO = mk(0.0f, 0.0f, 0.0f), nD = nO, sD = nO;
            float4 sO = make_float4(0.0f, 0.0f, 0.0f, 0.0f);
            float extOpacity = 0.0f, shadowOpacity = 0.0f;
            DCRT_MCLK_INIT;
            shade_path<CAPS>(sc, fc, hit, dir, rng, flags, thr, li, T, L, lsr, terminate, hasShadow, nO, nD, sO, sD,
                             extOpacity, shadowOpacity DCRT_MCLK_ARGS);
            shadowHit = false;
            if (hasShadow) {
                HitRecord sh;
                shadowHit = trace_full<true, false>(sc, mk(sO.x, sO.y, sO.z), sD, sO.w, watertight, f2b, 0.0f, lds, shift, &sh);
                ++shadowRays;
            }
            if (terminate) {
                const uint32_t p = slot(pool.pixel, path);
                sample_at(so.samplePosition, p) = pixel_sample(fc, p);
                sample_at(so.sampleValue, p) = make_float4(L.x + (!shadowHit ? lsr.x : 0.0f), L.y + (!shadowHit ? lsr.y : 0.0f),
                                                           L.z + (!shadowHit ? lsr.z : 0.0f), 0.0f);
                if (so.debugRng) sample_at(so.debugRng, p) = make_uint4(rng.s0, rng.s1, rng.s2, rng.s3);
                slot(pool.flags, path) = kFlagIdle;
                break;
            }
            if (!trace_full<false, false>(sc, nO, nD, inf(), watertight, f2b, 0.0f, lds, shift, &hit)) {
// ... 1045 lines not shown
```

### directcomputeraytracing_amd/csrc/device/tracer.hip

```cpp
#include <hip/hip_runtime.h>
#include <hip/hip_ext.h>

#include <dlfcn.h>

#include <algorithm>
#include <cmath>
#include <cstdio>
#include <cstdlib>
#include <cstring>
#include <map>
#include <mutex>
#include <string>
#include <type_traits>
#include <limits>
#include <vector>

#include "../../../include/dcrt.h"
#include "../host/bvh_layout.h"
#include "../host/film_rows.h"
#include "kernels_impl.h"

namespace dcrt {
void SetLastError(const std::string& s);
int CheckFilterParams(const dcrt_filter_params& f);
// ... 149 lines not shown
    const char* e = std::getenv(name);
    return e ? std::atoi(e) : unset;
}
bool EnvFlag(const char* name, bool unset)
{
    const char* e = std::getenv(name);
    return e ? std::atoi(e) != 0 : unset;
}

struct CreateKnobs {
    bool mergedCasts = true;
    bool virtualStart = true;
    uint32_t drainPaths = 0;
    uint32_t refillLanes = 36, parkLanes = 24;
    bool tuneOverride = false;
    uint32_t controlGridMul = 2, materialGridMul = 4;
};
CreateKnobs ReadCreateKnobs()
{
    CreateKnobs k;
    k.mergedCasts = !EnvFlag("DCRT_SPLIT_CASTS", false);
    k.virtualStart = EnvFlag("DCRT_VIRTUAL_START", true);
    k.drainPaths = (uint32_t)std::max(0, EnvInt("DCRT_DRAIN_PATHS", 0));
    if (const char* tune = std::getenv("DCRT_TRAVERSAL_TUNE")) {
        unsigned r = 0, p = 0;
        if (std::sscanf(tune, "%u,%u", &r, &p) == 2 && r >= 1 && r <= 64 && p >= 1 && p <= 64) {
            k.refillLanes = r;
            k.parkLanes = p;
            k.tuneOverride = true;
        }
    }
    k.controlGridMul = (uint32_t)std::max(0, EnvInt("DCRT_CONTROL_GRID", (int)k.controlGridMul));
    k.materialGridMul = (uint32_t)std::max(0, EnvInt("DCRT_MATERIAL_GRID", (int)k.materialGridMul));
    return k;
}

#ifndef DCRT_CAST_LDS_RESERVE
#define DCRT_CAST_LDS_RESERVE 12288
#endif
struct UploadKnobs {
    uint32_t castBlock = 0;
    bool noLdsCache = false;
    int pairTraversal = -1;
    uint32_t topNodes = 4096;
    bool nodeQuads = true;
    bool identCast = true;
    int stackRing = -1;
    size_t castLdsReserve = DCRT_CAST_LDS_RESERVE;
    uint32_t skipRoot = 1;
    bool ldsTrim = true;
    bool flatCast = true;
    bool flatMerge = true;
    uint32_t shadowCells = dcrt::kCellDefaultRes;
    int castBlocksPerCU = 0;
    int castGridMul = 0;
};
UploadKnobs ReadUploadKnobs()
{
    UploadKnobs k;
    k.castBlock = (uint32_t)EnvInt("DCRT_CAST_BLOCK", 0);
    k.noLdsCache = EnvFlag("DCRT_NO_LDS_CACHE", false);
    if (std::getenv("DCRT_PAIR_TRAVERSAL")) k.pairTraversal = EnvFlag("DCRT_PAIR_TRAVERSAL", false) ? 1 : 0;
    k.topNodes = (uint32_t)EnvInt("DCRT_TOP_NODES", (int)k.topNodes);
    k.nodeQuads = EnvFlag("DCRT_NODE_QUADS", true);
    k.identCast = EnvFlag("DCRT_IDENT_CAST", true);
    k.stackRing = EnvInt("DCRT_STACK_RING", -1);
    if (std::getenv("DCRT_CAST_LDS_RESERVE")) k.castLdsReserve = (size_t)std::max(0, EnvInt("DCRT_CAST_LDS_RESERVE", 0));
    k.skipRoot = (uint32_t)std::max(0, std::min(16, EnvInt("DCRT_SKIP_ROOT", (int)k.skipRoot)));
    k.ldsTrim = EnvFlag("DCRT_LDS_TRIM", true);
    k.flatCast = EnvFlag("DCRT_FLAT_CAST", true);
    k.flatMerge = EnvFlag("DCRT_FLAT_MERGE", true);
    k.shadowCells = (uint32_t)std::max(0, std::min((int)dcrt::kCellMaxRes, EnvInt("DCRT_SHADOW_CELLS", (int)k.shadowCells)));
    k.castBlocksPerCU = EnvInt("DCRT_CAST_BLOCKS_PER_CU", 0);
    k.castGridMul = EnvInt("DCRT_CAST_GRID_MUL", 0);
    return k;
}

struct ShadingKnobs {
    bool materialGeneric = false;
    uint32_t materialLds = 16384;
    bool materialLdsPartial = true;
    uint32_t fusedShadow = 1;
    uint32_t shadingTables = kTableAll;
};
ShadingKnobs ReadShadingKnobs()
{
    ShadingKnobs k;
    k.materialGeneric = EnvFlag("DCRT_MATERIAL_GENERIC", false);
    k.materialLds = (uint32_t)std::max(0, EnvInt("DCRT_MATERIAL_LDS", (int)k.materialLds));
    k.materialLdsPartial = EnvFlag("DCRT_MATERIAL_LDS_PARTIAL", true);
    k.fusedShadow = (uint32_t)std::max(0, EnvInt("DCRT_FUSED_SHADOW", (int)k.fusedShadow));
    k.shadingTables = (uint32_t)std::max(0, EnvInt("DCRT_SHADING_TABLES", (int)k.shadingTables)) & kTableAll;
    return k;
}

size_t g_ldsPerCU = 163840;
constexpr size_t kLdsGranule = 1280;
int LdsResident(size_t lds, const void* kernel = nullptr)
{
    if (kernel) {
        hipFuncAttributes attr{};
        if (hipFuncGetAttributes(&attr, kernel) == hipSuccess) lds += attr.sharedSizeBytes;
    }
    return lds ? (int)(g_ldsPerCU / ((lds + kLdsGranule - 1) / kLdsGranule * kLdsGranule)) : 1 << 20;
}
int ResidentPerCU(const void* kernel, uint32_t block, size_t lds, int* out)
{
    int n = 0;
    HIPCHECK(hipOccupancyMaxActiveBlocksPerMultiprocessor(&n, kernel, (int)block, lds));
    *out = std::min(n, LdsResident(lds, kernel));
    return DCRT_OK;
}

struct CastLaunch {
    CastFn kernel;
    size_t lds;
    const DeviceScene& scene;
    uint32_t resident;
};

struct CastPlan {
    uint32_t block = 256;
    uint32_t perCU = 0;
    bool allCached = false;
    bool pair = false;
    bool ident = false;
    bool flat = false;
    uint32_t ringRows = 0;
    uint32_t cellsRes = 0;
    size_t ldsWholeStack = 0;
    size_t ldsRing = 0;
    size_t ldsFlat = 0;
    DeviceScene scene{};
    DeviceScene sceneRing{};
    DeviceScene sceneFlat{};
    uint32_t resident[2][2] = {};

    bool Cells(bool instr, bool opacity) const { return flat && !instr && !opacity && sceneFlat.shadowRes != 0u; }
    CastLaunch Launch(bool instr, bool opacity) const
    {
        const bool useFlat = flat && !instr && !opacity, useRing = ringRows != 0 && !instr && !opacity;
        const CastVariant v{ instr, opacity, allCached, pair, ident, useRing, useFlat, Cells(instr, opacity) };
        return { CastKernel(v), useFlat ? ldsFlat : useRing ? ldsRing : ldsWholeStack, useFlat ? sceneFlat : useRing ? sceneRing : scene,
                 resident[instr][opacity] };
    }
};

using MaterialFn = void (*)(PathPool, DeviceScene, const FrameConstants*, Counters*, const Counters*, const SampleOut*, ShadowInline);

struct MaterialPlan {
    uint32_t caps = kCapAll;
    uint32_t mode = 0;
    uint32_t materials = 0, lights = 0;
    MaterialLds lds{};
    uint32_t tables = 0;
    const float* dielRows = nullptr;
    const float4* triFrames = nullptr;
    const float* envProb = nullptr;
    const float* envRowCdf = nullptr;
    const float* envMarginal = nullptr;
    uint32_t fusedMask = 0;
    uint32_t drainGrid = 0;

    MaterialFn Kernel(bool probe, bool fused) const
    {
        const bool od = caps == kCapOpaqueDelta;
        if (caps == kCapAllEnvImportance && !fused) {
            if (probe) return material_kernel<kCapAllEnvImportance, 0, true>;
            switch (mode) {
            case 1: return material_kernel<kCapAllEnvImportance, 1>;
            case 2: return material_kernel<kCapAllEnvImportance, 2>;
            default: return material_kernel<kCapAllEnvImportance, 0>;
            }
        }
        if (probe) return material_kernel<kCapAll, 0, true>;
        if (fused) return od ? material_kernel<kCapOpaqueDelta, 1, false, true> : material_kernel<kCapAll, 1, false, true>;
        switch (mode) {
        case 1: return od ? material_kernel<kCapOpaqueDelta, 1> : material_kernel<kCapAll, 1>;
        case 2: return od ? material_kernel<kCapOpaqueDelta, 2> : material_kernel<kCapAll, 2>;
        default: return od ? material_kernel<kCapOpaqueDelta, 0> : material_kernel<kCapAll, 0>;
        }
    }
    auto DrainKernel() const
    {
        return caps == kCapOpaqueDelta ? drain_kernel<kCapOpaqueDelta> : caps == kCapAllEnvImportance ? drain_kernel<kCapAllEnvImportance> : drain_kernel<kCapAll>;
    }
    using MegaFn = void (*)(DeviceScene, const FrameConstants*, Film, Globals*, uint32_t);
    MegaFn Megakernel(bool opacity) const
    {
        if (caps == kCapAllEnvImportance) return opacity ? megakernel<true, kCapAllEnvImportance> : megakernel<false, kCapAllEnvImportance>;
        return opacity ? megakernel<true> : megakernel<false>;
    }
    size_t LdsBytes(bool probe, bool fused) const { return probe ? 0u : lds.Bytes(fused); }
    void Apply(DeviceScene* d) const
    {
        d->ldsMaterials = materials;
        d->ldsLights = lights;
        d->shadingTables = tables;
        d->dielRows = dielRows;
        d->ldsRows = lds.rows ? materials : 0u;
        d->triFrames = triFrames;
        d->ldsFrames = lds.frames ? 1u : 0u;
        d->envProb = envProb;
        d->envRowCdf = envRowCdf;
        d->envMarginal = envMarginal;
    }
    bool BakedEquals(const MaterialPlan& o) const
    {
        return caps == o.caps && mode == o.mode && materials == o.materials && lights == o.lights && lds.shading == o.lds.shading &&
               lds.rows == o.lds.rows && lds.frames == o.lds.frames && lds.cells == o.lds.cells && tables == o.tables && drainGrid == o.drainGrid &&
               envProb == o.envProb && envRowCdf == o.envRowCdf && envMarginal == o.envMarginal;
    }
};

}

struct dcrt_tracer {
    int device = 0;
    hipStream_t stream = nullptr;
    bool ownsStream = false;
    uint32_t cuCount = 1;
    CreateKnobs knobs;
    uint32_t iterationsPerRender = kDefaultIterations;
    bool debugRng = false;
    int mode = 0;
    dcrt_output_params output{ DCRT_OUTPUT_PATH_TRACING, 20u };

    uint32_t poolSize = 0;
    uint32_t controlGrid = 0, materialGrid = 0;
    std::vector<void*> poolAllocs;
    PathPool pool{};
    float4* extRecs = nullptr;
    PathStateA* stateRecsA = nullptr;
    PathStateB* stateRecsB = nullptr;
    uint32_t* shadowHits = nullptr;
    FinishRec* finRecs = nullptr;
    uint32_t* finHits = nullptr;
    FrameConstants* dFrame = nullptr;
    Counters* dCounters = nullptr;
    Globals* dGlobals = nullptr;
    Counters* hCounters = nullptr;
    dcrt_bxdf_luts* dLuts = nullptr;

    std::vector<void*> sceneAllocs;
    bool hasScene = false;
    CastPlan plan;
    dcrt_upload_stats uploadStats{};
    MaterialPlan material;
    float* dDielRows = nullptr;
    float4* dTriFrames = nullptr;
    int envSampling = DCRT_ENV_SAMPLING_UNIFORM;
    float* dEnvProb = nullptr;
    float* dEnvRowCdf = nullptr;
    float* dEnvMarginal = nullptr;
    float envBuildMs = 0.0f;
    bool EnvTableActive() const { return hasScene && envSampling == DCRT_ENV_SAMPLING_IMPORTANCE && dEnvProb != nullptr; }
    bool FusedShadow() const
    {
        return material.lds.cells != 0u && !rowProbe && plan.Cells(instrCounters, (frame.features & DCRT_FEATURE_ALLOW_ANYHIT) != 0);
    }
    dcrt_material* dMaterials = nullptr;
    dcrt_light* dLights = nullptr;
    uint32_t* dInstanceFlags = nullptr;
    std::vector<dcrt_material> hostMaterials;
    std::vector<dcrt_light> hostLights;
    uint64_t* dCells = nullptr;
    uint32_t* dCellLeaves = nullptr;
    ShadowCells cells;
    std::vector<dcrt_bvh_node> cellNodes;
    std::vector<dcrt_vertex> cellVertices;
    std::vector<uint32_t> cellTriangles;
    std::vector<dcrt_float4x3> cellTransforms;
    uint32_t megaResident = 0;
    uint32_t viewResident = 0;
    uint32_t viewResidentOpacity = 0;

    std::vector<void*> filmAllocs, sampleAllocs, rowAllocs;
    Film film{};
    uint32_t filmW = 0, filmH = 0;
    uint32_t rowCount = 0;
    uint32_t bandCount = 0;
    dcrt_film_partition partition{ 1, 0, 64, 0 };
    std::vector<uint32_t> bands;
    uint32_t sampleImages = 0;
    uint32_t batchImages = 0;
    uint32_t lastSlot = 0;
    uint32_t seedStride = 1;
    bool keptSlots = false;
    uint32_t keptImages = 0;
    SampleOut* dSampleOut = nullptr;
    SampleOut hSampleOut = {};
    void** dSourceLists = nullptr;
    uint32_t sourceCap = 0;
    FilterConsts* dFilter = nullptr;
// ... 342 lines not shown
static int ValidateMaterials(const dcrt_material* materials, uint32_t count)
{
    if (!materials || count == 0) { SetLastError("no materials"); return DCRT_E_INVALID_ARG; }
    return DCRT_OK;
}
static int ValidateLights(const dcrt_light* lights, uint32_t count)
{
    if (count > DCRT_MAX_LIGHT_COUNT) { SetLastError("more than 5000 lights"); return DCRT_E_LIMIT; }
    if (!lights && count) { SetLastError("no light array"); return DCRT_E_INVALID_ARG; }
    return DCRT_OK;
}
static int ValidateInstanceFlags(const uint32_t* flags, uint32_t count)
{
    if (!flags || count == 0) { SetLastError("no instance flags"); return DCRT_E_INVALID_ARG; }
    return DCRT_OK;
}

static int KeepsResident(MaterialFn before, size_t a, MaterialFn after, size_t b, bool cap, bool* keeps)
{
    int ra = 0, rb = 0;
    CHECKED(ResidentPerCU((const void*)before, kMaterialBlock, a, &ra));
    CHECKED(ResidentPerCU((const void*)after, kMaterialBlock, b, &rb));
    *keeps = *keeps && rb >= ra && rb > 0 && (!cap || b <= 65536);
    return DCRT_OK;
}

int dcrt_tracer::PlanMaterial(const MaterialPlan* before, MaterialPlan* out)
{
    const ShadingKnobs k = ReadShadingKnobs();
    const DeviceScene& scene = plan.scene;
    const uint32_t T = scene.triangleCount, I = scene.instanceCount;
    const uint32_t M = (uint32_t)hostMaterials.size(), L = (uint32_t)hostLights.size();
    MaterialPlan p;
    uint32_t sceneCaps = scene.envCube ? kCapEnvCube : 0u;
    bool readsRows = false;
    for (const dcrt_material& m : hostMaterials) {
        const uint32_t type = m.flags & DCRT_MATERIAL_FLAG_TYPE_MASK;
        sceneCaps |= type <= DCRT_MATERIAL_TYPE_THIN_DIELECTRIC ? (1u << type) : kCapAll;
        if (m.flags & DCRT_MATERIAL_FLAG_MULTISCATTERING) sceneCaps |= kCapMultiscatter;
        if (m.albedo_texture_index != -1 || (m.flags & DCRT_MATERIAL_FLAG_ROUGHNESS_TEXTURE)) sceneCaps |= kCapTextures;
        readsRows = readsRows || (type == DCRT_MATERIAL_TYPE_PLASTIC && !(m.flags & DCRT_MATERIAL_FLAG_ROUGHNESS_TEXTURE));
    }
    for (const dcrt_light& l : hostLights) sceneCaps |= (l.flags & 0xFu) << kCapLightShift;
    p.caps = (sceneCaps & ~kCapOpaqueDelta) == 0u && !k.materialGeneric ? kCapOpaqueDelta : kCapAll;
    if (envSampling == DCRT_ENV_SAMPLING_IMPORTANCE && dEnvProb && scene.envCube && (sceneCaps & kCapLightEnv)) {
        p.caps = kCapAllEnvImportance;
        p.envProb = dEnvProb;
        p.envRowCdf = dEnvRowCdf;
        p.envMarginal = dEnvMarginal;
    }
    const bool counts = T > 0 && T < (1u << 20) && I < (1u << 20) && M < (1u << 20) && L < (1u << 20);
    const uint64_t whole = material_lds_layout(T, I, M, L, 0u, false, 0u, false).shading;
    const uint64_t rest = material_lds_layout(0u, I, M, L, 0u, false, 0u, false).shading;
    p.mode = !counts ? 0u : whole <= k.materialLds ? 1u : (k.materialLdsPartial && rest <= k.materialLds ? 2u : 0u);
    p.materials = p.mode ? M : 0u;
    p.lights = p.mode ? L : 0u;
    auto layout = [&](uint32_t rowMaterials, bool frames, bool cells) {
        return p.mode ? material_lds_layout(p.mode == 1u ? T : 0u, I, M, L, rowMaterials, frames, plan.sceneFlat.cachedNodes, cells) : MaterialLds{};
    };
    auto grow = [&](const MaterialLds& bigger, bool* taken) {
        *taken = true;
        for (const bool fused : { false, true })
            if (!fused || p.lds.cells) CHECKED(KeepsResident(p.Kernel(false, fused), p.lds.Bytes(fused), p.Kernel(false, fused), bigger.Bytes(fused), true, taken));
        if (*taken) p.lds = bigger;
        return (int)DCRT_OK;
    };
    p.lds = layout(0u, false, false);
    p.fusedMask = k.fusedShadow > 1u ? k.fusedShadow - 1u : 0u;
    if (k.fusedShadow && plan.flat && plan.cellsRes && p.mode == 1u) {
        const MaterialLds fused = layout(0u, false, true);
        bool fits = fused.cells <= k.materialLds;
        if (fits) CHECKED(KeepsResident(p.Kernel(false, false), p.lds.Bytes(false), p.Kernel(false, true), fused.Bytes(true), false, &fits));
        if (fits) p.lds = fused;
    }
    p.tables = k.shadingTables;
    if (!dDielRows || !readsRows) p.tables &= ~kTableDielRows;
    bool taken = false;
    if ((p.tables & kTableDielRows) && p.mode != 0u) CHECKED(grow(layout(M, false, p.lds.cells != 0u), &taken));
    if (!dTriFrames || p.mode != 1u || caps_any_scene(p.caps)) p.tables &= ~kTableFrames;
    if (p.tables & kTableFrames) {
        CHECKED(grow(layout(p.lds.rows ? M : 0u, true, p.lds.cells != 0u), &taken));
        if (!taken) p.tables &= ~kTableFrames;
    }
    p.dielRows = (p.tables & kTableDielRows) ? dDielRows : nullptr;
    p.triFrames = (p.tables & kTableFrames) ? dTriFrames : nullptr;
    if (before && before->caps == p.caps) {
        p.drainGrid = before->drainGrid;
    } else {
        int perCU = 0;
        CHECKED(ResidentPerCU((const void*)p.DrainKernel(), plan.block, plan.ldsWholeStack, &perCU));
        p.drainGrid = (uint32_t)std::max(1, perCU) * cuCount;
    }
    *out = p;
    return DCRT_OK;
}

int dcrt_tracer::ApplyMaterialPlan(const MaterialPlan& p)
{
    material = p;
    for (DeviceScene* d : { &plan.scene, &plan.sceneFlat, &plan.sceneRing }) material.Apply(d);
    if (material.tables & kTableDielRows) CHECKED(BuildDielRows());
    return DCRT_OK;
}

int dcrt_tracer::BuildDielRows()
{
    const uint32_t materialCount = (uint32_t)hostMaterials.size(), n = materialCount * kDielRowFloats;
    hipLaunchKernelGGL(build_diel_rows_kernel, dim3((n + 255) / 256), dim3(256), 0, stream, (const dcrt_material*)dMaterials, materialCount,
                       (const uint16_t*)dLuts->brdf_dielectric, (const uint16_t*)dLuts->brdf_dielectric_avg, dDielRows);
    HIPCHECK(hipGetLastError());
    return DCRT_OK;
}

int dcrt_tracer::RederiveShading()
{
    MaterialPlan next;
    CHECKED(PlanMaterial(&material, &next));
    if (next.fusedMask != material.fusedMask) newImage = true;
    const bool baked = next.BakedEquals(material);
    CHECKED(ApplyMaterialPlan(next));
    if (!baked) {
        HIPCHECK(hipStreamSynchronize(stream));
        InvalidateGraph();
    }
    return DCRT_OK;
}

int dcrt_tracer::UpdateMaterials(const dcrt_material* materials, uint32_t count)
{
    Annotation an("UpdateMaterials");
    if (!hasScene) { SetLastError("no scene uploaded"); return DCRT_E_NO_SCENE; }
    CHECKED(ValidateMaterials(materials, count));
    if (count != hostMaterials.size()) { SetLastError("material count differs from the uploaded scene's"); return DCRT_E_INVALID_ARG; }
    HIPCHECK(hipStreamSynchronize(stream));
    hostMaterials.assign(materials, materials + count);
    HIPCHECK(hipMemcpyAsync(dMaterials, hostMaterials.data(), (size_t)count * sizeof(dcrt_material), hipMemcpyHostToDevice, stream));
    uploadStats.shading_bytes += (uint64_t)count * sizeof(dcrt_material);
    ++uploadStats.material_updates;
    CHECKED(RederiveShading());
    HIPCHECK(hipStreamSynchronize(stream));
    return DCRT_OK;
}

int dcrt_tracer::UpdateLights(const dcrt_light* lights, uint32_t count)
{
    Annotation an("UpdateLights");
    if (!hasScene) { SetLastError("no scene uploaded"); return DCRT_E_NO_SCENE; }
    CHECKED(ValidateLights(lights, count));
    HIPCHECK(hipStreamSynchronize(stream));
    if (count) hostLights.assign(lights, lights + count);
    else hostLights.clear();
    if (count) HIPCHECK(hipMemcpyAsync(dLights, hostLights.data(), (size_t)count * sizeof(dcrt_light), hipMemcpyHostToDevice, stream));
    uploadStats.shading_bytes += (uint64_t)count * sizeof(dcrt_light);
    ++uploadStats.light_updates;
    CHECKED(RederiveShading());
    CHECKED(RebuildShadowCells());
    HIPCHECK(hipStreamSynchronize(stream));
    return DCRT_OK;
}

int dcrt_tracer::UpdateInstanceFlags(const uint32_t* flags, uint32_t count)
{
    Annotation an("UpdateInstanceFlags");
    if (!hasScene) { SetLastError("no scene uploaded"); return DCRT_E_NO_SCENE; }
    CHECKED(ValidateInstanceFlags(flags, count));
    if (count != plan.scene.instanceCount) { SetLastError("instance count differs from the uploaded scene's"); return DCRT_E_INVALID_ARG; }
// ... 1889 lines not shown
    const size_t tiles = (size_t)((t->filmW + T - 1) / T) * ((t->filmH + T - 1) / T);
    if (out_pixel)
        HIPCHECK(hipMemcpyAsync(out_pixel, t->noisePixelMap, (size_t)t->filmW * t->filmH * sizeof(float), hipMemcpyDeviceToHost, t->stream));
    if (out_tile) HIPCHECK(hipMemcpyAsync(out_tile, t->noiseTileMap, tiles * sizeof(float), hipMemcpyDeviceToHost, t->stream));
    HIPCHECK(hipStreamSynchronize(t->stream));
    return DCRT_OK;
}

DCRT_API int dcrt_tracer_render_converged(dcrt_tracer* t, uint32_t first_seed, const dcrt_converge_params* p,
                                          const dcrt_filter_params* f, dcrt_noise_stats* out_stats, int* out_converged)
{
    TRACER_GUARD(t);
    if (!p || !f || !out_stats || !out_converged) return DCRT_E_INVALID_ARG;
    return t->RenderConverged(first_seed, *p, *f, out_stats, out_converged);
}

DCRT_API int dcrt_tracer_set_adaptive(dcrt_tracer* t, int enable)
{
    TRACER_GUARD(t);
    return t->SetAdaptive(enable != 0);
}

DCRT_API int dcrt_tracer_set_sample_blocks(dcrt_tracer* t, const uint32_t* blocks, uint32_t count)
{
    TRACER_GUARD(t);
    return t->SetSampleBlocks(blocks, count);
}

DCRT_API int dcrt_tracer_get_sample_blocks(dcrt_tracer* t, uint32_t* out, uint32_t capacity, uint32_t* out_count)
{
    TRACER_GUARD(t);
    return t->GetSampleBlocks(out, capacity, out_count);
}

DCRT_API int dcrt_tracer_update_sample_blocks(dcrt_tracer* t, float threshold, uint32_t margin, uint32_t* out_active)
{
    TRACER_GUARD(t);
    return t->UpdateSampleBlocks(threshold, margin, out_active);
}

DCRT_API int dcrt_tracer_sample_blocks_device(dcrt_tracer* t, uint32_t width, uint32_t height, const void* d_film, const void* d_half,
                                              float threshold, uint32_t margin, void* d_flags, void* d_list, uint32_t* out_count)
{
    TRACER_GUARD(t);
    return t->SampleBlocks(width, height, (const float4*)d_film, (const float4*)d_half, threshold, margin, (uint32_t*)d_flags,
                           (uint32_t*)d_list, out_count, nullptr);
}

DCRT_API int dcrt_tracer_adaptive_timings(dcrt_tracer* t, float* out_mask_ms, float* out_compact_ms, float* out_fill_ms)
{
    TRACER_GUARD(t);
    if (!out_mask_ms || !out_compact_ms || !out_fill_ms) return DCRT_E_INVALID_ARG;
    *out_mask_ms = *out_compact_ms = *out_fill_ms = 0.0f;
    HIPCHECK(hipStreamSynchronize(t->stream));
    if (t->adMaskTimed) {
        HIPCHECK(hipEventElapsedTime(out_mask_ms, t->adEvents[0], t->adEvents[1]));
        HIPCHECK(hipEventElapsedTime(out_compact_ms, t->adEvents[1], t->adEvents[2]));
    }
    if (t->adFillTimed) HIPCHECK(hipEventElapsedTime(out_fill_ms, t->adEvents[3], t->adEvents[4]));
    return DCRT_OK;
}

DCRT_API int dcrt_tracer_render_adaptive(dcrt_tracer* t, uint32_t first_seed, const dcrt_converge_params* p, uint32_t margin,
                                         const dcrt_filter_params* f, dcrt_noise_stats* out_stats, int* out_converged,
                                         dcrt_adaptive_report* out_report)
{
    TRACER_GUARD(t);
    if (!p || !f || !out_stats || !out_converged) return DCRT_E_INVALID_ARG;
    return t->RenderAdaptive(first_seed, *p, margin, *f, out_stats, out_converged, out_report);
}

DCRT_API int dcrt_tracer_counters(dcrt_tracer* t, dcrt_ray_stats* out)
{
    TRACER_GUARD(t);
    if (!out) return DCRT_E_INVALID_ARG;
    Globals g;
    HIPCHECK(hipMemcpyAsync(&g, t->dGlobals, sizeof(Globals), hipMemcpyDeviceToHost, t->stream));
    HIPCHECK(hipStreamSynchronize(t->stream));
    out->extension_rays = g.extRays;
    out->shadow_rays = g.shadowRays;
    out->new_paths = t->imagesCompleted * (uint64_t)t->rowCount * t->filmW - t->pathsSkipped;
    out->iterations = g.iterations;
    out->images_completed = t->imagesCompleted;
    return DCRT_OK;
}

DCRT_API int dcrt_tracer_set_instrumentation(dcrt_tracer* t, int counters, int ext_timing)
{
    TRACER_GUARD(t);
    if ((counters != 0) != t->instrCounters) t->InvalidateGraph();
    t->instrCounters = counters != 0;
    t->extTiming = ext_timing != 0;
    return DCRT_OK;
}

DCRT_API int dcrt_tracer_get_info(dcrt_tracer* t, dcrt_tracer_info* out)
{
    TRACER_GUARD(t);
    if (!out) return DCRT_E_INVALID_ARG;
    const CastPlan& plan = t->plan;
    const CastLaunch shipped = plan.Launch(false, false);
    out->path_pool_size = t->poolSize;
    out->scene_in_lds = t->hasScene && plan.allCached ? 1u : 0u;
    out->cached_nodes = t->hasScene ? plan.scene.cachedNodes : 0u;
    out->cached_triangles = t->hasScene ? plan.scene.cachedTris : 0u;
    out->cast_block = plan.block;
    out->traversal_stack = t->hasScene ? plan.scene.stackSize : 0u;
    out->material_generic = caps_any_scene(t->material.caps) ? 1u : 0u;
    out->pair_traversal = t->hasScene && plan.pair ? 1u : 0u;
    out->control_grid = t->controlGrid;
    out->material_grid = t->materialGrid;
    out->cast_grid = shipped.resident;
    out->material_lds = t->material.lds.shading;
    out->cast_identity = plan.ident ? (plan.flat ? 2u : 1u) : 0u;
    out->stack_lds_rows = t->hasScene ? shipped.scene.stackRows : 0u;
    out->ring_rows = t->hasScene ? plan.ringRows : 0u;
    out->cast_waves_per_cu = plan.perCU * (plan.block / 64u);
    const bool cells = t->hasScene && shipped.scene.shadowRes != 0u;
    out->shadow_cells = cells ? shipped.scene.shadowRes : 0u;
    out->shadow_cell_max_leaves = cells ? t->cells.maxLeaves : 0u;
    out->shadow_cell_mean_leaves = cells ? t->cells.meanLeaves : 0.0f;
    out->shadow_inline = t->hasScene && t->FusedShadow() ? 1u : 0u;
    out->shading_tables = t->hasScene ? t->material.tables : 0u;
    out->dielectric_row_bytes = t->hasScene && (t->material.tables & kTableDielRows) ? diel_rows_bytes((uint32_t)t->hostMaterials.size()) : 0u;
    out->dielectric_row_lds = t->hasScene ? t->material.lds.rows : 0u;
    out->frame_table_bytes = t->hasScene ? t->material.lds.frames : 0u;
    return DCRT_OK;
}

DCRT_API int dcrt_tracer_debug_ring_spills(dcrt_tracer* t, uint64_t* out)
{
    TRACER_GUARD(t);
    if (!out) return DCRT_E_INVALID_ARG;
    *out = 0;
    const CastLaunch shipped = t->plan.Launch(false, false);
    if (!t->hasScene || !shipped.scene.spill) return DCRT_OK;
    const size_t n = (size_t)shipped.resident * t->plan.block * shipped.scene.stackSize;
    std::vector<uint32_t> h(n);
    HIPCHECK(hipStreamSynchronize(t->stream));
    HIPCHECK(hipMemcpy(h.data(), shipped.scene.spill, n * 4, hipMemcpyDeviceToHost));
    for (const uint32_t w : h) *out += w != 0u;
    return DCRT_OK;
}

DCRT_API int dcrt_tracer_traversal_stats(dcrt_tracer* t, dcrt_traversal_stats* out)
{
    TRACER_GUARD(t);
    if (!out) return DCRT_E_INVALID_ARG;
    unsigned long long v[8];
    HIPCHECK(hipMemcpyAsync(v, t->dInstr, sizeof(v), hipMemcpyDeviceToHost, t->stream));
    HIPCHECK(hipStreamSynchronize(t->stream));
    CHECKED(t->CollectTimes());
    out->ext_node_visits = v[0]; out->ext_triangle_tests = v[1]; out->ext_blas_entries = v[2];
    out->shadow_node_visits = v[3]; out->shadow_triangle_tests = v[4]; out->shadow_blas_entries = v[5];
    out->ext_launches = t->kindLaunches[dcrt_tracer::kTimedCast];
    out->ext_kernel_ms = t->kindMs[dcrt_tracer::kTimedCast];
    out->ext_max_node_visits = v[6]; out->shadow_max_node_visits = v[7];
    out->material_launches = t->kindLaunches[dcrt_tracer::kTimedMaterial];
    out->material_kernel_ms = t->kindMs[dcrt_tracer::kTimedMaterial];
    out->control_launches = t->kindLaunches[dcrt_tracer::kTimedControl];
    out->control_kernel_ms = t->kindMs[dcrt_tracer::kTimedControl];
    return DCRT_OK;
}

DCRT_API int dcrt_tracer_reset_stats(dcrt_tracer* t)
{
    TRACER_GUARD(t);
    HIPCHECK(hipStreamSynchronize(t->stream));
    HIPCHECK(hipMemsetAsync(t->dInstr, 0, 8 * sizeof(unsigned long long), t->stream));
    Globals g;
    HIPCHECK(hipMemcpyAsync(&g, t->dGlobals, sizeof(Globals), hipMemcpyDeviceToHost, t->stream));
    HIPCHECK(hipStreamSynchronize(t->stream));
    g.extRays = g.shadowRays = g.iterations = 0;
    t->imagesCompleted = 0;
    t->pathsSkipped = 0;
    HIPCHECK(hipMemcpyAsync(t->dGlobals, &g, sizeof(Globals), hipMemcpyHostToDevice, t->stream));
    HIPCHECK(hipStreamSynchronize(t->stream));
    t->eventsUsed = 0;
    for (int k = 0; k < dcrt_tracer::kTimedKinds; ++k) {
        t->kindMs[k] = 0.0;
        t->kindLaunches[k] = 0;
    }
    return DCRT_OK;
}

DCRT_API int dcrt_tracer_synchronize(dcrt_tracer* t)
{
    TRACER_GUARD(t);
    HIPCHECK(hipStreamSynchronize(t->stream));
    return DCRT_OK;
}

DCRT_API int dcrt_tracer_get_luts(dcrt_tracer* t, dcrt_bxdf_luts* out)
{
    TRACER_GUARD(t);
    if (!out) return DCRT_E_INVALID_ARG;
    HIPCHECK(hipMemcpyAsync(out, t->dLuts, sizeof(dcrt_bxdf_luts), hipMemcpyDeviceToHost, t->stream));
    HIPCHECK(hipStreamSynchronize(t->stream));
    return DCRT_OK;
}

DCRT_API int dcrt_tracer_set_luts(dcrt_tracer* t, const dcrt_bxdf_luts* luts)
{
    TRACER_GUARD(t);
    if (!luts) return DCRT_E_INVALID_ARG;
    HIPCHECK(hipMemcpyAsync(t->dLuts, luts, sizeof(dcrt_bxdf_luts), hipMemcpyHostToDevice, t->stream));
    HIPCHECK(hipStreamSynchronize(t->stream));
    if (t->hasScene && (t->material.tables & kTableDielRows)) {
        CHECKED(t->BuildDielRows());
        HIPCHECK(hipStreamSynchronize(t->stream));
    }
    return DCRT_OK;
}

static int TraceBatch(dcrt_tracer* t, const dcrt_ray* d_rays, uint32_t n, dcrt_ray_hit* d_hits, uint32_t* d_occ, bool any, uint32_t features)
{
    if (!t->hasScene) { SetLastError("no scene uploaded"); return DCRT_E_NO_SCENE; }
    const CastPlan& plan = t->plan;
    const uint32_t grid = std::min<uint32_t>((n + plan.block - 1) / plan.block, plan.resident[0][0]);
    if (n == 0) return DCRT_OK;
    unsigned long long* instr = t->instrCounters ? t->dInstr : nullptr;
    auto kernel = any ? (instr ? batch_trace_kernel<true, true> : batch_trace_kernel<true, false>)
                      : (instr ? batch_trace_kernel<false, true> : batch_trace_kernel<false, false>);
    hipLaunchKernelGGL(kernel, dim3(grid), dim3(plan.block), plan.ldsWholeStack, t->stream, plan.scene, d_rays, n, features, d_hits, d_occ, instr);
    HIPCHECK(hipGetLastError());
    return DCRT_OK;
}

DCRT_API int dcrt_tracer_trace_rays(dcrt_tracer* t, const dcrt_ray* rays, uint32_t n, dcrt_ray_hit* out, uint32_t features)
{
    TRACER_GUARD(t);
    if ((!rays || !out) && n) return DCRT_E_INVALID_ARG;
    std::vector<void*> tmp;
    dcrt_ray* dr = nullptr; dcrt_ray_hit* dh = nullptr;
    CHECKED(DeviceAlloc(&dr, n, &tmp));
    CHECKED(DeviceAlloc(&dh, n, &tmp));
    int rc = DCRT_OK;
    if (hipMemcpyAsync(dr, rays, (size_t)n * sizeof(dcrt_ray), hipMemcpyHostToDevice, t->stream) != hipSuccess) rc = DCRT_E_HIP;
    if (rc == DCRT_OK) rc = TraceBatch(t, dr, n, dh, nullptr, false, features);
    if (rc == DCRT_OK && hipMemcpyAsync(out, dh, (size_t)n * sizeof(dcrt_ray_hit), hipMemcpyDeviceToHost, t->stream) != hipSuccess) rc = DCRT_E_HIP;
    if (hipStreamSynchronize(t->stream) != hipSuccess) rc = DCRT_E_HIP;
    FreeAll(&tmp);
    return rc;
}

DCRT_API int dcrt_tracer_occluded(dcrt_tracer* t, const dcrt_ray* rays, uint32_t n, uint32_t* out, uint32_t features)
{
    TRACER_GUARD(t);
    if ((!rays || !out) && n) return DCRT_E_INVALID_ARG;
    std::vector<void*> tmp;
    dcrt_ray* dr = nullptr; uint32_t* dOcc = nullptr;
    CHECKED(DeviceAlloc(&dr, n, &tmp));
    CHECKED(DeviceAlloc(&dOcc, n, &tmp));
    int rc = DCRT_OK;
    if (hipMemcpyAsync(dr, rays, (size_t)n * sizeof(dcrt_ray), hipMemcpyHostToDevice, t->stream) != hipSuccess) rc = DCRT_E_HIP;
    if (rc == DCRT_OK) rc = TraceBatch(t, dr, n, nullptr, dOcc, true, features);
// ... 609 lines not shown
```

### include/dcrt.h

```cpp
#ifndef DCRT_H_
#define DCRT_H_

#include <stdint.h>
#include <stddef.h>

#ifdef __cplusplus
extern "C" {
#endif

#define DCRT_API __attribute__((visibility("default")))

#define DCRT_OK              0
#define DCRT_E_INVALID_ARG  -1
#define DCRT_E_HIP          -2
#define DCRT_E_NO_SCENE     -3
#define DCRT_E_IO           -4
#define DCRT_E_LIMIT        -5
#define DCRT_E_NO_DEVICE    -6

#define DCRT_LIGHT_INDEX_INVALID        0xFFFFFFFFu
#define DCRT_LIGHT_FLAGS_POINT_LIGHT        0x1u
#define DCRT_LIGHT_FLAGS_MESH_LIGHT         0x2u
#define DCRT_LIGHT_FLAGS_DIRECTIONAL_LIGHT  0x4u
#define DCRT_LIGHT_FLAGS_ENVIRONMENT_LIGHT  0x8u
// ... 84 lines not shown
    const uint32_t* instance_flags;
    const uint32_t* instance_material_overrides;
    const dcrt_material* materials;         uint32_t material_count;
    const dcrt_light* lights;               uint32_t light_count;
    uint32_t environment_light_index;
    const dcrt_texture* textures;           uint32_t texture_count;
    const float* env_cube_rgb;              uint32_t env_cube_size;
    uint32_t bvh_traversal_stack_size;
} dcrt_flat_scene;

#define DCRT_LUT_BRDF_COUNT            (32 * 32)
#define DCRT_LUT_BRDF_AVG_COUNT        (32)
#define DCRT_LUT_BRDF_DIELECTRIC_COUNT (32 * 16 * 32)
#define DCRT_LUT_BRDF_DIELECTRIC_AVG_COUNT (16 * 16 * 2)
#define DCRT_LUT_BSDF_COUNT            (32 * 16 * 32)
#define DCRT_LUT_BSDF_AVG_COUNT        (16 * 16 * 2)
typedef struct dcrt_bxdf_luts {
    uint16_t brdf[DCRT_LUT_BRDF_COUNT];
    uint16_t brdf_avg[DCRT_LUT_BRDF_AVG_COUNT];
    uint16_t brdf_dielectric[DCRT_LUT_BRDF_DIELECTRIC_COUNT];
    uint16_t brdf_dielectric_avg[DCRT_LUT_BRDF_DIELECTRIC_AVG_COUNT];
    uint16_t bsdf[DCRT_LUT_BSDF_COUNT];
    uint16_t bsdf_avg[DCRT_LUT_BSDF_AVG_COUNT];
} dcrt_bxdf_luts;

typedef struct dcrt_frame_params {
    float camera_transform[16];
    uint32_t resolution[2];
    float film_size[2];
    float aperture_radius;
    float focal_distance;
    float film_distance;
    uint32_t blade_count;
    float blade_vertex_pos[2];
    float aperture_base_angle;
    uint32_t frame_seed;
    uint32_t max_bounce_count;
    uint32_t light_count;
    uint32_t environment_light_index;
    uint32_t features;
} dcrt_frame_params;

#define DCRT_FILTER_BOX      0
#define DCRT_FILTER_TRIANGLE 1
#define DCRT_FILTER_GAUSSIAN 2
#define DCRT_FILTER_MITCHELL 3
#define DCRT_FILTER_LANCZOS  4
typedef struct dcrt_filter_params {
    uint32_t filter;
    float radius;
    float gaussian_alpha;
    float mitchell_b;
    float mitchell_c;
    uint32_t lanczos_tau;
} dcrt_filter_params;

typedef struct dcrt_ray {
    float origin[3];
    float t_max;
    float direction[3];
    float t_min;
} dcrt_ray;
typedef struct dcrt_ray_hit {
    float t;
    float u, v;
    uint32_t triangle_id;
    uint32_t instance_index;
} dcrt_ray_hit;

typedef struct dcrt_tracer_config {
    uint32_t path_pool_size;
    uint32_t iterations_per_render;
    int32_t device;
    void* stream;
    uint32_t debug_rng;
} dcrt_tracer_config;

typedef struct dcrt_ray_stats {
    uint64_t extension_rays;
    uint64_t shadow_rays;
    uint64_t new_paths;
    uint64_t iterations;
    uint64_t images_completed;
} dcrt_ray_stats;

typedef struct dcrt_film_partition {
    uint32_t world_size;
    uint32_t rank;
    uint32_t stripe_height;
    uint32_t halo_rows;
} dcrt_film_partition;

typedef struct dcrt_traversal_stats {
    uint64_t ext_node_visits, ext_triangle_tests, ext_blas_entries;
    uint64_t shadow_node_visits, shadow_triangle_tests, shadow_blas_entries;
    uint64_t ext_launches;
    double ext_kernel_ms;
    uint64_t ext_max_node_visits, shadow_max_node_visits;
    uint64_t material_launches;
    double material_kernel_ms;
    uint64_t control_launches;
    double control_kernel_ms;
} dcrt_traversal_stats;

typedef struct dcrt_tracer_info {
    uint32_t path_pool_size;
    uint32_t scene_in_lds;
    uint32_t cached_nodes, cached_triangles;
    uint32_t cast_block;
    uint32_t traversal_stack;
    uint32_t material_generic;
    uint32_t pair_traversal;
    uint32_t control_grid, material_grid;
    uint32_t cast_grid;
    uint32_t material_lds;
    uint32_t cast_identity;
    uint32_t stack_lds_rows;
    uint32_t ring_rows;
    uint32_t cast_waves_per_cu;
    uint32_t shadow_cells;
    uint32_t shadow_cell_max_leaves;
    float shadow_cell_mean_leaves;
    uint32_t shadow_inline;
    uint32_t shading_tables;
    uint32_t dielectric_row_bytes;
    uint32_t dielectric_row_lds;
    uint32_t frame_table_bytes;
} dcrt_tracer_info;

typedef struct dcrt_tracer dcrt_tracer;
typedef struct dcrt_scene dcrt_scene;

#define DCRT_ABI_VERSION 5
DCRT_API int dcrt_abi_version(void);
DCRT_API const char* dcrt_version(void);
DCRT_API const char* dcrt_last_error(void);
DCRT_API int dcrt_device_count(int* out_count);

DCRT_API int dcrt_scene_create(dcrt_scene** out_scene);
DCRT_API void dcrt_scene_destroy(dcrt_scene* scene);
DCRT_API int dcrt_scene_reset(dcrt_scene* scene, uint32_t resolution_width, uint32_t resolution_height);
DCRT_API int dcrt_scene_load_from_file(dcrt_scene* scene, const char* path);
DCRT_API int dcrt_scene_add_punctual_light(dcrt_scene* scene, const float position[3], const float euler_angles[3],
                                           const float color[3], int is_directional);
DCRT_API int dcrt_scene_set_punctual_light(dcrt_scene* scene, uint32_t index, const float position[3],
                                           const float euler_angles[3], const float color[3], int is_directional);
DCRT_API int dcrt_scene_remove_punctual_light(dcrt_scene* scene, uint32_t index);
DCRT_API int dcrt_scene_remove_environment_light(dcrt_scene* scene);
#define DCRT_DIRTY_LIGHTS          0x01u
#define DCRT_DIRTY_MATERIALS       0x02u
#define DCRT_DIRTY_INSTANCE_FLAGS  0x04u
#define DCRT_DIRTY_CAMERA          0x08u
#define DCRT_DIRTY_SCENE           0x10u
DCRT_API int dcrt_scene_acquire_dirty(dcrt_scene* scene, uint32_t* out_bits);
DCRT_API int dcrt_scene_flatten(dcrt_scene* scene);
DCRT_API int dcrt_scene_set_environment_light(dcrt_scene* scene, const float color[3],
                                              const float* cube_rgb, uint32_t cube_size);
DCRT_API int dcrt_scene_set_camera(dcrt_scene* scene, const float position[3], const float euler_angles[3]);
DCRT_API int dcrt_scene_set_lens(dcrt_scene* scene, int camera_type, float fov_x, float focal_length,
                                 float focal_distance, float relative_aperture, uint32_t blade_count,
                                 float aperture_rotation, const float film_size[2]);
DCRT_API int dcrt_scene_set_max_bounce(dcrt_scene* scene, uint32_t max_bounce);
DCRT_API int dcrt_scene_set_filter(dcrt_scene* scene, const dcrt_filter_params* filter);
DCRT_API int dcrt_scene_get_filter(const dcrt_scene* scene, dcrt_filter_params* out_filter);
DCRT_API int dcrt_scene_get_resolution(const dcrt_scene* scene, uint32_t* width, uint32_t* height);
DCRT_API int dcrt_scene_get_material_count(const dcrt_scene* scene, uint32_t* out_count);
DCRT_API int dcrt_scene_set_material(dcrt_scene* scene, uint32_t index, int material_type, const float albedo[3],
                                     float roughness, const float ior[3], const float k[3],
                                     int multiscattering, int two_sided);
typedef struct dcrt_material_setting {
    float albedo[3];
    float roughness;
    float ior[3];
    float opacity;
    float k[3];
    float tiling[2];
    uint32_t material_type;
    int32_t albedo_texture_index;
    int32_t opacity_texture_index;
    uint32_t internal_scattering_mode;
    uint32_t multiscattering;
    uint32_t is_two_sided;
    uint32_t has_roughness_texture;
} dcrt_material_setting;
DCRT_API int dcrt_scene_get_material_setting(const dcrt_scene* scene, uint32_t index, dcrt_material_setting* out_setting);
DCRT_API int dcrt_scene_set_material_multiscattering(dcrt_scene* scene, uint32_t index, int enable);
DCRT_API int dcrt_scene_set_material_opacity(dcrt_scene* scene, uint32_t index, float opacity,
                                             int32_t opacity_texture_index);
DCRT_API int dcrt_scene_set_features(dcrt_scene* scene, uint32_t features);
DCRT_API int dcrt_scene_get_features(const dcrt_scene* scene, uint32_t* out_features);
DCRT_API int dcrt_scene_get_flat(dcrt_scene* scene, dcrt_flat_scene* out_flat);
DCRT_API int dcrt_scene_get_frame_params(const dcrt_scene* scene, uint32_t frame_seed, dcrt_frame_params* out_params);
DCRT_API int dcrt_scene_get_bvh_info(const dcrt_scene* scene, uint32_t* tlas_nodes, uint32_t* total_nodes,
                                     uint32_t* max_stack_size);

typedef struct dcrt_obj_mesh dcrt_obj_mesh;
DCRT_API int dcrt_scene_get_content_counts(const dcrt_scene* scene, uint32_t* out_meshes, uint32_t* out_instances);
DCRT_API int dcrt_scene_get_loaded_mesh(dcrt_scene* scene, uint32_t mesh, dcrt_obj_mesh* out_mesh);
DCRT_API int dcrt_scene_get_instance(const dcrt_scene* scene, uint32_t instance, uint32_t* out_mesh_index,
                                     float out_transform[12]);

typedef struct dcrt_scene_settings {
    uint32_t resolution[2];
    uint32_t max_bounce_count;
    uint32_t camera_type;
    float fov_x, focal_length, focal_distance, relative_aperture;
    uint32_t aperture_blade_count;
    float aperture_rotation;
    float film_size[2];
    float camera_position[3];
    float camera_euler_angles[3];
    uint32_t features;
    uint32_t has_environment_light;
    float environment_color[3];
    const float* env_cube_rgb;
    uint32_t env_cube_size;
// ... 246 lines not shown
```

Measured before the change: 19430 Mrays/s.

## Finish last-bounce paths early in material kernel and recycle slots by epoch

When a path's next extension ray would exceed the max bounce and the scene has no mesh or environment lights, the material kernel now writes the path's sample and frees its slot right away. It no longer waits for another trace-and-shade round trip. The final ray is still appended to a reverse-filled region of the extension queue and traced, but its hit is discarded. Freed slots carry an epoch tag so the control kernel reuses them only after a safe iteration boundary. This aims to shorten each path's lifetime in the wavefront pipeline and keep the pool fuller with new paths. The cost is extra counters, epoch bookkeeping and traversal of rays whose results are unused.

Result: faster. 19670 Mrays/s (median of 6 runs) (+1.2%).

```diff
diff --git a/directcomputeraytracing_amd/_abi.py b/directcomputeraytracing_amd/_abi.py
--- a/directcomputeraytracing_amd/_abi.py
+++ b/directcomputeraytracing_amd/_abi.py
@@ -8,7 +8,7 @@
 LIB_PATH = PKG_DIR / "libdcrt.so"
 
 DCRT_OK = 0
-ABI_VERSION = 5
+ABI_VERSION = 6
 ERRORS = {-1: "DCRT_E_INVALID_ARG", -2: "DCRT_E_HIP", -3: "DCRT_E_NO_SCENE", -4: "DCRT_E_IO",
           -5: "DCRT_E_LIMIT", -6: "DCRT_E_NO_DEVICE"}
 LIGHT_INDEX_INVALID = 0xFFFFFFFF
@@ -142,7 +142,7 @@
 
 class RayStats(C.Structure):
     _fields_ = [("extension_rays", C.c_uint64), ("shadow_rays", C.c_uint64), ("new_paths", C.c_uint64),
-                ("iterations", C.c_uint64), ("images_completed", C.c_uint64)]
+                ("iterations", C.c_uint64), ("images_completed", C.c_uint64), ("early_finished", C.c_uint64)]
 
 
 class FilmPartition(C.Structure):
@@ -167,7 +167,8 @@
                 ("cast_identity", C.c_uint32), ("stack_lds_rows", C.c_uint32), ("ring_rows", C.c_uint32),
                 ("cast_waves_per_cu", C.c_uint32), ("shadow_cells", C.c_uint32), ("shadow_cell_max_leaves", C.c_uint32),
                 ("shadow_cell_mean_leaves", C.c_float), ("shadow_inline", C.c_uint32), ("shading_tables", C.c_uint32),
-                ("dielectric_row_bytes", C.c_uint32), ("dielectric_row_lds", C.c_uint32), ("frame_table_bytes", C.c_uint32)]
+                ("dielectric_row_bytes", C.c_uint32), ("dielectric_row_lds", C.c_uint32), ("frame_table_bytes", C.c_uint32),
+                ("early_finish", C.c_uint32)]
 
 
 class ShadowCellsInfo(C.Structure):
diff --git a/directcomputeraytracing_amd/csrc/device/dscene.h b/directcomputeraytracing_amd/csrc/device/dscene.h
--- a/directcomputeraytracing_amd/csrc/device/dscene.h
+++ b/directcomputeraytracing_amd/csrc/device/dscene.h
@@ -26,6 +26,7 @@
 constexpr uint32_t kCapMaterialsMask = 0x1Fu;
 constexpr uint32_t kCapLightShift = 7;
 constexpr uint32_t kCapOpaqueDelta = kCapMatDiffuse | kCapMatPlastic | kCapMatConductor | kCapLightPoint | kCapLightDirectional;
+constexpr bool caps_early_finish(uint32_t caps) { return (caps & (kCapLightMesh | kCapLightEnv)) == 0u; }
 
 template <uint32_t CAPS>
 DEV void assume_light_caps(uint32_t flags)
@@ -87,6 +88,7 @@
     const float* envProb;
     const float* envRowCdf;
     const float* envMarginal;
+    uint32_t earlyFinish;
 };
 
 constexpr uint32_t kTableDeltaPdf = 1u << 0;
diff --git a/directcomputeraytracing_amd/csrc/device/kernels.h b/directcomputeraytracing_amd/csrc/device/kernels.h
--- a/directcomputeraytracing_amd/csrc/device/kernels.h
+++ b/directcomputeraytracing_amd/csrc/device/kernels.h
@@ -12,6 +12,13 @@
 constexpr uint32_t kFlagFirst = 0x08000000u;
 constexpr uint32_t kFlagShadowPending = 0x04000000u;
 constexpr uint32_t kFlagShadowResolved = 0x02000000u;
+constexpr uint32_t kFlagIdleFrom = 0x40000000u;
+constexpr uint32_t kEpochMask = 0x3FFFFFFFu;
+DEV uint32_t idle_from(uint32_t epoch) { return kFlagIdleFrom | (epoch & kEpochMask); }
+DEV bool slot_idle(uint32_t flags, uint32_t epoch)
+{
+    return (flags & kFlagIdle) != 0u || ((flags & kFlagIdleFrom) != 0u && ((epoch - flags) & kEpochMask) < (kEpochMask >> 1));
+}
 constexpr uint32_t kBlockW = 8, kBlockH = 8;
 #ifndef DCRT_CONTROL_BLOCK
 #define DCRT_CONTROL_BLOCK 256
@@ -31,17 +38,29 @@
 constexpr uint32_t kNoPixel = 0xFFFFFFFFu;
 constexpr uint32_t kDrainedWord = kCounterWords + 1;
 constexpr uint32_t kInlineShadowWord = kCounterWords + 2;
-constexpr uint32_t kCounterLines = kCounterWords + 2 + kShards;
+constexpr uint32_t kLastRayWord = kInlineShadowWord + kShards;
+constexpr uint32_t kCounterLines = kLastRayWord + kShards;
+constexpr uint32_t kEpochLine = kCounterLines;
 constexpr uint32_t kEntryFirst = 0x80000000u;
 
 struct Counters {
-    uint32_t w[kCounterLines * kShardStride];
-};
+    uint32_t w[(kCounterLines + 1) * kShardStride];
+};
+DEV uint32_t epoch_of(const Counters* c) { return c->w[kEpochLine * kShardStride]; }
 DEV uint32_t inline_shadow_rays(const Counters* c)
 {
     uint32_t t = 0;
     for (uint32_t s = 0; s < kShards; ++s) t += c->w[(kInlineShadowWord + s) * kShardStride];
     return t;
+}
+DEV unsigned long long* last_ctr(Counters* c, uint32_t s) { return (unsigned long long*)(c->w + (kLastRayWord + s) * kShardStride); }
+DEV void last_totals(const Counters* c, uint32_t* rays, uint32_t* completed)
+{
+    *rays = *completed = 0u;
+    for (uint32_t s = 0; s < kShards; ++s) {
+        *rays += c->w[(kLastRayWord + s) * kShardStride];
+        *completed += c->w[(kLastRayWord + s) * kShardStride + 1u];
+    }
 }
 DEV uint32_t virtual_items(const Counters* c) { return c->w[kVirtualWord * kShardStride]; }
 DEV bool drained(const Counters* c) { return c->w[kDrainedWord * kShardStride] != 0u; }
@@ -60,6 +79,7 @@
     uint32_t skipFilm;
     uint32_t filmImageBase;
     unsigned long long extRays, shadowRays, iterations;
+    unsigned long long earlyFinished;
 };
 
 DEV uint32_t* qctr(Counters* c, uint32_t q, uint32_t s) { return c->w + (q * kShards + s) * kShardStride; }
@@ -105,6 +125,28 @@
         base = ge ? m.prefix[k] : base;
     }
     return s * cap + (i - base);
+}
+DEV uint32_t last_total(const Counters* c)
+{
+    uint32_t t = 0;
+    for (uint32_t s = 0; s < kShards; ++s) t += c->w[(kLastRayWord + s) * kShardStride];
+    return t;
+}
+DEV uint32_t last_pos(const Counters* c, uint32_t cap, uint32_t j)
+{
+    uint32_t s = 0, base = 0, run = 0;
+    const uint32_t* w = c->w;
+#if defined(__HIP_DEVICE_COMPILE__)
+    asm volatile("" : "+s"(w));
+#endif
+#pragma unroll
+    for (uint32_t k = 0; k + 1 < kShards; ++k) {
+        run += w[(kLastRayWord + k) * kShardStride];
+        const bool ge = j >= run;
+        s += ge ? 1u : 0u;
+        base = ge ? run : base;
+    }
+    return s * cap + (cap - 1u - (j - base));
 }
 DEV float4* ext_rec(float4* recs, uint32_t q) { return (float4*)((char*)recs + (uint64_t)(q * 32u)); }
 DEV const float4* ext_rec(const float4* recs, uint32_t q) { return (const float4*)((const char*)recs + (uint64_t)(q * 32u)); }
@@ -213,6 +255,7 @@
     float4 liLsr;
     float4 lsrSlot;
 };
+constexpr uint32_t kFinishEarly = 1u;
 constexpr uint32_t kDestFinish = 0x80000000u;
 
 struct PathPool {
diff --git a/directcomputeraytracing_amd/csrc/device/kernels_impl.h b/directcomputeraytracing_amd/csrc/device/kernels_impl.h
--- a/directcomputeraytracing_amd/csrc/device/kernels_impl.h
+++ b/directcomputeraytracing_amd/csrc/device/kernels_impl.h
@@ -260,6 +260,7 @@
 {
     __shared__ uint32_t sm[64];
     if (g->stopped) return;
+    const uint32_t epoch = epoch_of(cnt);
     {
         QueueMapN<kFinShards> fm;
         qmap(prev, kQFinish, &fm);
@@ -277,7 +278,7 @@
             const uint32_t p = slot(pool.pixel, path);
             sample_at(film.samplePosition, p) = pixel_sample(*fc, p);
             sample_at(film.sampleValue, p) = make_float4(li.x, li.y, li.z, 0.0f);
-            slot(pool.flags, path) = kFlagIdle;
+            slot(pool.flags, path) = asu(fr.lsrSlot.w) == kFinishEarly ? idle_from(epoch + 1u) : kFlagIdle;
         }
     }
     const uint32_t lane = threadIdx.x & 63u;
@@ -309,7 +310,7 @@
     for (uint32_t base = blockIdx.x * blockDim.x; base < pool.size; base += gridDim.x * blockDim.x) {
     const uint32_t tid = base + threadIdx.x;
     const uint32_t vb = base / kControlBlock;
-    const bool idle = (pool.flags[tid] & kFlagIdle) != 0;
+    const bool idle = slot_idle(pool.flags[tid], epoch);
     const bool waveIdle = __ballot(!idle) == 0ull;
     uint32_t claimed = 0;
     bool got = false;
@@ -456,6 +457,7 @@
                                                                              const Counters* prev, const SampleOut* __restrict__ sampleOut, ShadowInline si)
 {
     static_assert(!FUSED || (SCENE_LDS == 1 && !PROBE), "FUSED: beside the whole LDS shading copy");
+    constexpr bool EARLY = caps_early_finish(CAPS) && !PROBE;
 #if defined(DCRT_MATERIAL_PRIO) && DCRT_MATERIAL_PRIO > 0
     __builtin_amdgcn_s_setprio(DCRT_MATERIAL_PRIO);
 #endif
@@ -524,6 +526,8 @@
     DCRT_MCLK_INIT;
     uint32_t itemsDone = 0;
     uint32_t round = 0;
+    uint32_t doneFlag = kFlagIdle;
+    if constexpr (EARLY) doneFlag = (uint32_t)__builtin_amdgcn_readfirstlane((int)idle_from(epoch_of(cnt) + 2u));
     for (uint32_t base = blockIdx.x * blockDim.x; base < count; base += gridDim.x * blockDim.x) {
     const uint32_t i = base + threadIdx.x;
     bool active = i < count;
@@ -532,7 +536,7 @@
         newPixel = slot(pool.pixel, i);
         active = newPixel != kNoPixel;
     }
-    bool terminate = false, hasShadow = false, ends = false;
+    bool terminate = false, hasShadow = false, ends = false, last = false;
     uint32_t path = 0, pix = 0;
     float4 sample = make_float4(0.0f, 0.0f, 0.0f, 0.0f);
     float2* outPos = nullptr;
@@ -604,6 +608,11 @@
             if (hasShadow) slot(pool.shadowOpacity, out) = shadowOpacity;
         }
         ends = terminate && !hasShadow;
+        if constexpr (EARLY) {
+            const uint32_t mode = sc.earlyFinish;
+            last = !terminate && (flags & 0xFFu) > fcv.maxBounce && mode != 0u && (mode != 2u || (path & 1u) == 0u) &&
+                   (fcv.features & DCRT_FEATURE_ALLOW_ANYHIT) == 0u;
+        }
         if constexpr (PROBE) {
             uint32_t* rowRays = sampleOut->rowRays;
             const uint32_t p = virt ? newPixel : slot(pool.pixel, out);
@@ -616,10 +625,10 @@
         sL = L;
         sLsr = lsr;
         sRng = make_uint4(rng.s0, rng.s1, rng.s2, rng.s3);
-        if (ends || terminate) {
+        if (ends || terminate || last) {
             const SampleOut so = *sampleOut;
-            if (ends || so.debugRng) pix = slot(pool.pixel, out);
-            if (ends) {
+            if (ends || last || so.debugRng) pix = slot(pool.pixel, out);
+            if (ends || last) {
                 sample = make_float4(L.x + 0.0f, L.y + 0.0f, L.z + 0.0f, 0.0f);
                 outPos = so.samplePosition;
                 outVal = so.sampleValue;
@@ -639,20 +648,41 @@
     const bool queued = active && hasShadow && !inlined;
     DCRT_MCLK(5);
     uint32_t es, ss;
-    const bool fin = active && terminate && hasShadow;
+    const bool done = last && (!hasShadow || inlined);
+    if (done) {
+        sample.x = (sL.x + (!occluded ? sLsr.x : 0.0f)) + 0.0f;
+        sample.y = (sL.y + (!occluded ? sLsr.y : 0.0f)) + 0.0f;
+        sample.z = (sL.z + (!occluded ? sLsr.z : 0.0f)) + 0.0f;
+    }
+    const bool fin = active && ((terminate && hasShadow) || (last && !done));
     uint32_t fb;
-    block_append3(active && !terminate, qctr(cnt, kQExt, shard), queued, qctr(cnt, kQShadow, shard),
+    uint32_t lastBase = 0u, lastRank = 0u;
+    if constexpr (EARLY) {
+        const unsigned long long lm = __ballot(last);
+        if (lm != 0ull) {
+            lastRank = __builtin_amdgcn_mbcnt_hi((uint32_t)(lm >> 32), __builtin_amdgcn_mbcnt_lo((uint32_t)lm, 0u));
+            const unsigned long long both = (unsigned long long)__popcll(lm) | ((unsigned long long)__popcll(__ballot(done)) << 32);
+            if ((threadIdx.x & 63u) == 0u) lastBase = (uint32_t)atomicAdd(last_ctr(cnt, shard), both);
+        }
+    }
+    block_append3(active && !terminate && !last, qctr(cnt, kQExt, shard), queued, qctr(cnt, kQShadow, shard),
                   fin, qctr(cnt, kQFinish, fshard), sm + (round & 1u) * 48u, &es, &ss, &fb);
     DCRT_MCLK(6);
+    if constexpr (EARLY) lastBase = (uint32_t)__builtin_amdgcn_readfirstlane((int)lastBase);
     const uint32_t qNext = shard * pool.recCap + es;
     const uint32_t fPos = fshard * pool.finCap + fb;
     asm volatile("" ::"v"(pix));
-    if (ends) {
+    if (ends || done) {
         store_global(outPos, pix, pixel_sample(fcv, pix));
         store_global(outVal, pix, sample);
-        slot(pool.flags, path) = kFlagIdle;
-    }
-    if (active && !terminate) {
+        slot(pool.flags, path) = done ? doneFlag : kFlagIdle;
+    }
+    if (last) {
+        float4* r = ext_rec(pool.extRec, shard * pool.recCap + (pool.recCap - 1u - (lastBase + lastRank)));
+        r[0] = make_float4(nO.x, nO.y, nO.z, 0.0f);
+        r[1] = make_float4(nD.x, nD.y, nD.z, asf(path));
+    }
+    if (active && !terminate && !last) {
         float4* r = ext_rec(pool.extRec, qNext);
         r[0] = make_float4(nO.x, nO.y, nO.z, 0.0f);
         r[1] = make_float4(nD.x, nD.y, nD.z, asf(path));
@@ -666,14 +696,14 @@
     if (fin) {
         FinishRec& fr = pool.finRec[fPos];
         fr.liLsr = make_float4(sL.x, sL.y, sL.z, sLsr.x);
-        fr.lsrSlot = make_float4(sLsr.y, sLsr.z, asf(path), 0.0f);
+        fr.lsrSlot = make_float4(sLsr.y, sLsr.z, asf(path), asf(last ? kFinishEarly : 0u));
         if (inlined) pool.finHit[fPos] = occluded ? 1u : 0u;
     }
     if (queued) {
         const uint32_t sq = shard * pool.recCap + ss;
         float4* r = ext_rec(pool.shRec, sq);
         r[0] = sO;
-        r[1] = make_float4(sD.x, sD.y, sD.z, asf(terminate ? (fPos | kDestFinish) : qNext));
+        r[1] = make_float4(sD.x, sD.y, sD.z, asf(terminate || last ? (fPos | kDestFinish) : qNext));
         if (fcv.features & DCRT_FEATURE_ALLOW_ANYHIT) slot(pool.shadowQueue, sq) = path;
     }
     DCRT_MCLK(2);
@@ -722,6 +752,7 @@
 
 
 constexpr uint32_t kNoItem = 0xFFFFFFFFu;
+constexpr uint32_t kLastItem = 0xFFFFFFFEu;
 #ifndef DCRT_INLINE_ENTRY
 #define DCRT_INLINE_ENTRY 1
 #endif
@@ -899,18 +930,19 @@
     scene_cache_load(sc, stackMem, block_shift());
     QueueMap qm;
     qmap(cnt, kQExt, &qm);
+    const uint32_t nExt = qm.prefix[kShards];
     TraversalStats st = {};
     persistent_trace<false, INSTR, OPACITY>(
-        sc, qm.prefix[kShards], fc->features, fc->refillLanes, fc->parkLanes, stackMem + threadIdx.x, block_shift(),
-        [&](uint32_t i) __attribute__((always_inline)) { return qpos(pool.recCap, qm, i); },
+        sc, nExt + last_total(cnt), fc->features, fc->refillLanes, fc->parkLanes, stackMem + threadIdx.x, block_shift(),
+        [&](uint32_t i) __attribute__((always_inline)) { return i >= nExt ? last_pos(cnt, pool.recCap, i - nExt) : qpos(pool.recCap, qm, i); },
         [&](uint32_t i, uint32_t q, TravState& s) __attribute__((always_inline)) {
             const float4* r = ext_rec((const float4*)pool.extRec, q);
             const float4 o = r[0], d = r[1];
             trav_init(s, mk(o.x, o.y, o.z), mk(d.x, d.y, d.z), 0.0f, inf());
             if (OPACITY) s.opacitySample = pool.extOpacity[asu(d.w) & ~kEntryFirst];
-            return i;
+            return i >= nExt ? kLastItem : i;
         },
-        [&](uint32_t item, const TravState& s) __attribute__((always_inline)) { emit_hit(pool, item, s); },
+        [&](uint32_t item, const TravState& s) __attribute__((always_inline)) { if (item != kLastItem) emit_hit(pool, item, s); },
         st, DCRT_WAVE_TAG(g));
     if (INSTR) flush_stats(st, instr);
     (void)g;
@@ -920,20 +952,29 @@
 {
     if (blockIdx.x == 0) {
         if (threadIdx.x == 0) {
+#if defined(__HIP_DEVICE_COMPILE__)
+            asm volatile("" : "+s"(cnt));
+#endif
             uint32_t fin = 0;
             for (uint32_t sh = 0; sh < kFinShards; ++sh) fin += qctr_load(cnt, kQFinish, sh);
             const uint32_t virt = virtual_items(cnt);
-            const uint32_t ext = virt ? virt : qtotal(cnt, kQExt);
+            uint32_t lastRays, completed;
+            last_totals(cnt, &lastRays, &completed);
+            const uint32_t queued = virt ? virt : qtotal(cnt, kQExt);
+            const uint32_t ext = queued + lastRays;
             if (!virt) g->extRays += ext;
+            g->earlyFinished += lastRays;
+            nextCnt->w[kEpochLine * kShardStride] = epoch_of(cnt) + 1u;
             g->shadowRays += shadowRays + inline_shadow_rays(cnt);
             g->iterations += 1ull;
             g->staticFill = 0u;
             const bool idle = g->prevLive == 0u && ext == 0u;
             g->poolIdle = idle ? 1u : 0u;
             g->imageComplete = (idle && !g->stopped) ? 1u : 0u;
-            g->prevLive = ext + fin;
+            g->prevLive = queued + fin + completed;
         }
         if (threadIdx.x < kCounterLines) nextCnt->w[threadIdx.x * kShardStride] = 0u;
+        if (threadIdx.x < kShards) nextCnt->w[(kLastRayWord + threadIdx.x) * kShardStride + 1u] = 0u;
     }
 }
 
@@ -984,7 +1025,7 @@
     QueueMap qe, qs;
     qmap(cnt, kQExt, &qe);
     qmap(cnt, kQShadow, &qs);
-    const uint32_t nExt = qe.prefix[kShards], nShadow = qs.prefix[kShards];
+    const uint32_t nExt = qe.prefix[kShards], nShadow = qs.prefix[kShards], nClosest = nExt + last_total(cnt);
     const uint32_t* shQueue = sgpr_ptr(pool.shadowQueue);
     const float4* extRec = sgpr_ptr((const float4*)pool.extRec);
     const float4* shRec = sgpr_ptr((const float4*)pool.shRec);
@@ -1036,25 +1077,26 @@
 #endif
         if (!DCRT_CELLS_LAST) shadowSection();
         persistent_trace<false, INSTR, OPACITY, false, ALL_CACHED, PAIR, kLayout, IDENT, RING, FLAT>(
-            sc, nExt, fc->features, fc->refillLanes, fc->parkLanes, stackMem + threadIdx.x, block_shift(),
-            [&](uint32_t i) __attribute__((always_inline)) { return qpos(pool.recCap, qe, i); },
+            sc, nClosest, fc->features, fc->refillLanes, fc->parkLanes, stackMem + threadIdx.x, block_shift(),
+            [&](uint32_t i) __attribute__((always_inline)) { return i >= nExt ? last_pos(cnt, pool.recCap, i - nExt) : qpos(pool.recCap, qe, i); },
             [&](uint32_t i, uint32_t v, TravState& s) __attribute__((always_inline)) {
                 const float4* r = ext_rec(extRec, v);
                 const float4 o = r[0], d = r[1];
                 trav_init(s, mk(o.x, o.y, o.z), mk(d.x, d.y, d.z), 0.0f, inf());
-                return i;
+                return i >= nExt ? kLastItem : i;
             },
-            [&](uint32_t item, const TravState& s) __attribute__((always_inline)) { emit_hit(pool, item, s); },
+            [&](uint32_t item, const TravState& s) __attribute__((always_inline)) { if (item != kLastItem) emit_hit(pool, item, s); },
             st, DCRT_WAVE_TAG(g));
         if (DCRT_CELLS_LAST) shadowSection();
     } else {
     persistent_trace<false, INSTR, OPACITY, true, ALL_CACHED, PAIR, kLayout, IDENT, RING, FLAT>(
-        sc, nExt + nShadow, fc->features, fc->refillLanes, fc->parkLanes, stackMem + threadIdx.x, block_shift(),
+        sc, nClosest + nShadow, fc->features, fc->refillLanes, fc->parkLanes, stackMem + threadIdx.x, block_shift(),
         [&](uint32_t i) __attribute__((always_inline)) {
-            return i >= nExt ? qpos(pool.recCap, qs, i - nExt) : qpos(pool.recCap, qe, i);
+            if (i >= nClosest) return qpos(pool.recCap, qs, i - nClosest);
+            return i >= nExt ? last_pos(cnt, pool.recCap, i - nExt) : qpos(pool.recCap, qe, i);
         },
         [&](uint32_t i, uint32_t v, TravState& s) __attribute__((always_inline)) {
-            const bool shadow = i >= nExt;
+            const bool shadow = i >= nClosest;
             const float4* r = ext_rec(shadow ? shRec : extRec, v);
             const float4 o = r[0], d = r[1];
             trav_init(s, mk(o.x, o.y, o.z), mk(d.x, d.y, d.z), 0.0f, shadow ? o.w : inf());
@@ -1064,11 +1106,11 @@
                 s.opacitySample = shadow ? pool.shadowOpacity[path] : pool.extOpacity[path];
             }
             if (INSTR) st = TraversalStats{};
-            return shadow ? asu(d.w) : i;
+            return shadow ? asu(d.w) : (i >= nExt ? kLastItem : i);
         },
         [&](uint32_t item, const TravState& s) __attribute__((always_inline)) {
             if (s.anyHit) emit_occlusion(pool, item, s);
-            else emit_hit(pool, item, s);
+            else if (item != kLastItem) emit_hit(pool, item, s);
             if (INSTR) {
                 TraversalStats& dst = s.anyHit ? stShadow : stExt;
                 dst.nodes += st.nodes; dst.tris += st.tris; dst.blas += st.blas;
@@ -1323,7 +1365,9 @@
     QueueMapN<kFinShards> fm;
     qmap(cnt, kQFinish, &fm);
     const uint32_t nExt = qe.prefix[kShards], nFin = fm.prefix[kFinShards];
-    if (nExt + nFin == 0u || nExt + nFin > fc.drainPaths) return;
+    uint32_t lastRays, completed;
+    last_totals(cnt, &lastRays, &completed);
+    if (nExt + nFin + completed == 0u || nExt + nFin + completed > fc.drainPaths) return;
     for (uint32_t sh = 0; sh < kShards; ++sh) {
         const uint32_t blocks = g->totalBlocks > sh ? (g->totalBlocks - sh + kShards - 1) / kShards : 0u;
         if (__hip_atomic_load(&g->nextBlock[sh * kShardStride], __ATOMIC_RELAXED, __HIP_MEMORY_SCOPE_AGENT) < blocks) return;
diff --git a/directcomputeraytracing_amd/csrc/device/tracer.hip b/directcomputeraytracing_amd/csrc/device/tracer.hip
--- a/directcomputeraytracing_amd/csrc/device/tracer.hip
+++ b/directcomputeraytracing_amd/csrc/device/tracer.hip
@@ -255,6 +255,7 @@
     bool materialLdsPartial = true;
     uint32_t fusedShadow = 1;
     uint32_t shadingTables = kTableAll;
+    uint32_t earlyFinish = 1;
 };
 ShadingKnobs ReadShadingKnobs()
 {
@@ -264,6 +265,7 @@
     k.materialLdsPartial = EnvFlag("DCRT_MATERIAL_LDS_PARTIAL", true);
     k.fusedShadow = (uint32_t)std::max(0, EnvInt("DCRT_FUSED_SHADOW", (int)k.fusedShadow));
     k.shadingTables = (uint32_t)std::max(0, EnvInt("DCRT_SHADING_TABLES", (int)k.shadingTables)) & kTableAll;
+    k.earlyFinish = (uint32_t)std::max(0, std::min(2, EnvInt("DCRT_EARLY_FINISH", (int)k.earlyFinish)));
     return k;
 }
 
@@ -334,6 +336,8 @@
     const float* envMarginal = nullptr;
     uint32_t fusedMask = 0;
     uint32_t drainGrid = 0;
+    uint32_t earlyFinish = 0;
+    uint32_t EarlyFinish(bool probe, bool opacity) const { return probe || opacity ? 0u : earlyFinish; }
 
     MaterialFn Kernel(bool probe, bool fused) const
     {
@@ -377,12 +381,13 @@
         d->envProb = envProb;
         d->envRowCdf = envRowCdf;
         d->envMarginal = envMarginal;
+        d->earlyFinish = earlyFinish;
     }
     bool BakedEquals(const MaterialPlan& o) const
     {
         return caps == o.caps && mode == o.mode && materials == o.materials && lights == o.lights && lds.shading == o.lds.shading &&
                lds.rows == o.lds.rows && lds.frames == o.lds.frames && lds.cells == o.lds.cells && tables == o.tables && drainGrid == o.drainGrid &&
-               envProb == o.envProb && envRowCdf == o.envRowCdf && envMarginal == o.envMarginal;
+               envProb == o.envProb && envRowCdf == o.envRowCdf && envMarginal == o.envMarginal && earlyFinish == o.earlyFinish;
     }
 };
 
@@ -891,6 +896,7 @@
         CHECKED(grow(layout(p.lds.rows ? M : 0u, true, p.lds.cells != 0u), &taken));
         if (!taken) p.tables &= ~kTableFrames;
     }
+    p.earlyFinish = caps_early_finish(p.caps) ? k.earlyFinish : 0u;
     p.dielRows = (p.tables & kTableDielRows) ? dDielRows : nullptr;
     p.triFrames = (p.tables & kTableFrames) ? dTriFrames : nullptr;
     if (before && before->caps == p.caps) {
@@ -2946,6 +2952,7 @@
     out->new_paths = t->imagesCompleted * (uint64_t)t->rowCount * t->filmW - t->pathsSkipped;
     out->iterations = g.iterations;
     out->images_completed = t->imagesCompleted;
+    out->early_finished = g.earlyFinished;
     return DCRT_OK;
 }
 
@@ -2989,6 +2996,7 @@
     out->dielectric_row_bytes = t->hasScene && (t->material.tables & kTableDielRows) ? diel_rows_bytes((uint32_t)t->hostMaterials.size()) : 0u;
     out->dielectric_row_lds = t->hasScene ? t->material.lds.rows : 0u;
     out->frame_table_bytes = t->hasScene ? t->material.lds.frames : 0u;
+    out->early_finish = t->hasScene ? t->material.EarlyFinish(t->rowProbe, (t->frame.features & DCRT_FEATURE_ALLOW_ANYHIT) != 0) : 0u;
     return DCRT_OK;
 }
 
@@ -3035,7 +3043,7 @@
     Globals g;
     HIPCHECK(hipMemcpyAsync(&g, t->dGlobals, sizeof(Globals), hipMemcpyDeviceToHost, t->stream));
     HIPCHECK(hipStreamSynchronize(t->stream));
-    g.extRays = g.shadowRays = g.iterations = 0;
+    g.extRays = g.shadowRays = g.iterations = g.earlyFinished = 0;
     t->imagesCompleted = 0;
     t->pathsSkipped = 0;
     HIPCHECK(hipMemcpyAsync(t->dGlobals, &g, sizeof(Globals), hipMemcpyHostToDevice, t->stream));
diff --git a/include/dcrt.h b/include/dcrt.h
--- a/include/dcrt.h
+++ b/include/dcrt.h
@@ -190,6 +190,7 @@
     uint64_t new_paths;
     uint64_t iterations;
     uint64_t images_completed;
+    uint64_t early_finished;
 } dcrt_ray_stats;
 
 typedef struct dcrt_film_partition {
@@ -234,12 +235,13 @@
     uint32_t dielectric_row_bytes;
     uint32_t dielectric_row_lds;
     uint32_t frame_table_bytes;
+    uint32_t early_finish;
 } dcrt_tracer_info;
 
 typedef struct dcrt_tracer dcrt_tracer;
 typedef struct dcrt_scene dcrt_scene;
 
-#define DCRT_ABI_VERSION 5
+#define DCRT_ABI_VERSION 6
 DCRT_API int dcrt_abi_version(void);
 DCRT_API const char* dcrt_version(void);
 DCRT_API const char* dcrt_last_error(void);
```
